# thiery-lab/manifold-mcmc-for-diffusions

Hardware: AMD Instinct MI355X
Metric: constrained-leapfrog steps/sec (all chains), FHN noisy-obs 400 sub-steps (higher is better)
Workload: dtype f64; 1 GPU; FHN noisy-obs, T=100 obs, S=400 steps/obs, R=5 obs/subseq, sigma_y=0.1, 256 chains per GPU (BASELINE.json configs[1]), Newton solver, standard splitting; chains_per_gpu=256, global_chains=256, dim_q=80106, traj_len=16, stepping=chmc_leapfrog_steps per trajectory (batched steps), chain_steps_nominal=152320, parallelism=chains x1 (no data-path collective, 1 gather), ranks_joined=1, collective_world_size=1, collective_route=torch.distributed gather, overlap_halves=-1

## Files before the change

### manifold_mcmc_for_diffusions_amd/context.py

```python
import ctypes as C
import numpy as np
from . import _lib
from ._lib import ChmcConfig, as_c, ptr, iptr, check

MODEL_IDS = {"fhn": 0, "sir": 1, "fhn_nb": 2}
STATUS_NAMES = {0: "ok", 1: "not_converged", 2: "diverged", 3: "non_reversible", -1: "inactive"}


class ChmcContext:
    def __init__(self, model, obs_interval, num_steps_per_obs, num_obs_per_subseq, y_seq, sigma=None,
                 use_gaussian_splitting=False, num_chains=1, device=0):
        L = _lib.lib()
        self.L = L
        y = as_c(np.asarray(y_seq).reshape(-1))
        self._y = y
        cfg = ChmcConfig(
            model=MODEL_IDS[model] if isinstance(model, str) else int(model), num_obs=len(y),
            num_steps_per_obs=int(num_steps_per_obs),
            num_obs_per_subseq=0 if num_obs_per_subseq is None else int(num_obs_per_subseq),
            noisy=2 if isinstance(sigma, str) else int(sigma is not None),
            use_gaussian_splitting=int(bool(use_gaussian_splitting)),
            num_chains=int(num_chains), device=int(device), obs_interval=float(obs_interval),
            sigma=0.0 if sigma is None or isinstance(sigma, str) else float(sigma), y_seq=ptr(y))
        h = C.c_void_p()
# ... 197 lines not shown
        check(self.L.chmc_jacob_constr_blocks(self.h, ptr(du), ptr(dv)), "chmc_jacob_constr_blocks")
        return du, dv

    def chol_gram_blocks(self):
        cC = np.empty((self.B, self.U, self.U))
        cD = np.empty((self.B, self.num_blocks, self.RM, self.RM))
        check(self.L.chmc_chol_gram_blocks(self.h, ptr(cC), ptr(cD)), "chmc_chol_gram_blocks")
        return cC, cD

    def log_det_sqrt_gram(self):
        out = np.empty(self.B)
        check(self.L.chmc_log_det_sqrt_gram(self.h, ptr(out)), "chmc_log_det_sqrt_gram")
        return out

    def grad_log_det_sqrt_gram(self):
        g = np.empty((self.B, self.Q))
        check(self.L.chmc_grad_log_det_sqrt_gram(self.h, ptr(g)), "chmc_grad_log_det_sqrt_gram")
        return g

    def lmult_by_jacob_constr(self, vct):
        vct = self._bq(vct, "vct")
        out = np.empty((self.B, self.dim_c))
        check(self.L.chmc_lmult_by_jacob_constr(self.h, ptr(vct), ptr(out)), "chmc_lmult_by_jacob_constr")
        return out

    def _bc(self, a, name):
        a = as_c(a)
        if a.shape != (self.B, self.dim_c):
            raise ValueError(f"{name} must have shape ({self.B}, {self.dim_c}), got {a.shape}")
        return a

    def rmult_by_jacob_constr(self, lam):
        lam = self._bc(lam, "vct")
        out = np.empty((self.B, self.Q))
        check(self.L.chmc_rmult_by_jacob_constr(self.h, ptr(lam), ptr(out)), "chmc_rmult_by_jacob_constr")
        return out

    def lmult_by_inv_gram(self, vct):
        vct = self._bc(vct, "vct")
        out = np.empty((self.B, self.dim_c))
        check(self.L.chmc_lmult_by_inv_gram(self.h, ptr(vct), ptr(out)), "chmc_lmult_by_inv_gram")
        return out

    def normal_space_component(self, vct):
        vct = self._bq(vct, "vct")
        out = np.empty((self.B, self.Q))
        check(self.L.chmc_normal_space_component(self.h, ptr(vct), ptr(out)), "chmc_normal_space_component")
        return out

    def project_onto_cotangent_space(self):
        check(self.L.chmc_project_onto_cotangent_space(self.h), "chmc_project_onto_cotangent_space")

    def hamiltonian(self):
        h = np.empty((self.B, 3))
        check(self.L.chmc_hamiltonian(self.h, ptr(h)), "chmc_hamiltonian")
        return h

    def neg_log_dens_and_grad(self, q, use_gaussian_splitting=False, want_grad=True):
        QH = self.U + self.NV
        q = as_c(q)
        if q.shape != (self.B, QH):
            raise ValueError(f"q must have shape ({self.B}, {QH}), got {q.shape}")
        val = np.empty(self.B)
        g = np.empty((self.B, QH)) if want_grad else None
        check(self.L.chmc_neg_log_dens_and_grad(self.h, ptr(q), int(bool(use_gaussian_splitting)), ptr(val), ptr(g)),
              "chmc_neg_log_dens_and_grad")
        return val, g

    def neg_log_dens_and_grad_device(self, q_dev_ptr, grad_dev_ptr=None, use_gaussian_splitting=False):
        val = np.empty(self.B)
        check(self.L.chmc_neg_log_dens_and_grad_device(self.h, C.c_void_p(q_dev_ptr), int(bool(use_gaussian_splitting)),
                                                       ptr(val), C.c_void_p(grad_dev_ptr or 0)),
              "chmc_neg_log_dens_and_grad_device")
        return val

    def adam_objective_device(self, u_v_dev_ptr, grad_dev_ptr):
        out = np.empty((self.B, 3))
        check(self.L.chmc_adam_objective_device(self.h, C.c_void_p(u_v_dev_ptr), C.c_void_p(grad_dev_ptr), ptr(out)),
              "chmc_adam_objective_device")
        return out

    def adam_update_device(self, u_v_dev_ptr, m_dev_ptr, v_dev_ptr, grad_dev_ptr, coef, b1=0.9, b2=0.999, eps=1e-8):
        coef = as_c(np.asarray(coef, dtype=np.float64).reshape(self.B, 2))
        check(self.L.chmc_adam_update_device(self.h, C.c_void_p(u_v_dev_ptr), C.c_void_p(m_dev_ptr), C.c_void_p(v_dev_ptr),
                                             C.c_void_p(grad_dev_ptr), ptr(coef), float(b1), float(b2), float(eps)),
              "chmc_adam_update_device")

    def project(self, q, dt, newton=True, constraint_tol=1e-9, position_tol=1e-8, divergence_tol=1e10, max_iters=50):
        q = self._bq(q, "q")
        dt = as_c(np.broadcast_to(np.asarray(dt, dtype=np.float64), (self.B,)))
        q_out, mu = np.empty((self.B, self.Q)), np.empty((self.B, self.Q))
        iters, status = np.zeros(self.B, dtype=np.int32), np.zeros(self.B, dtype=np.int32)
        ndq, err = np.empty(self.B), np.empty(self.B)
        check(self.L.chmc_project(self.h, int(newton), ptr(q), ptr(dt), constraint_tol, position_tol, divergence_tol,
                                  int(max_iters), ptr(q_out), ptr(mu), iptr(iters), ptr(ndq), ptr(err), iptr(status)),
              "chmc_project")
        return dict(q=q_out, mu=mu, iters=iters, norm_dq=ndq, err=err, status=status)

    def leapfrog_step(self, dt, active=None, n_inner_step=1, newton=True, constraint_tol=1e-9, position_tol=1e-8,
                      divergence_tol=1e10, max_iters=50, reverse_check_tol=2e-8):
        dt = as_c(np.broadcast_to(np.asarray(dt, dtype=np.float64), (self.B,)))
        act = None if active is None else np.ascontiguousarray(active, dtype=np.int32)
        status = np.zeros(self.B, dtype=np.int32)
        itf, itb = np.zeros(self.B, dtype=np.int32), np.zeros(self.B, dtype=np.int32)
        rev = np.zeros(self.B)
        check(self.L.chmc_leapfrog_step(self.h, ptr(dt), iptr(act), int(n_inner_step), int(newton), constraint_tol,
                                        position_tol, divergence_tol, int(max_iters), reverse_check_tol, iptr(status),
                                        iptr(itf), iptr(itb), ptr(rev)), "chmc_leapfrog_step")
        return dict(status=status, iters_fwd=itf, iters_bwd=itb, rev_err=rev)

    def leapfrog_steps(self, dt, n_steps, active=None, n_inner_step=1, newton=True, constraint_tol=1e-9, position_tol=1e-8,
                       divergence_tol=1e10, max_iters=50, reverse_check_tol=2e-8):
        dt = as_c(np.broadcast_to(np.asarray(dt, dtype=np.float64), (self.B,)))
        act = None if active is None else np.ascontiguousarray(active, dtype=np.int32)
        per_chain = None if np.isscalar(n_steps) else np.ascontiguousarray(np.broadcast_to(n_steps, (self.B,)), dtype=np.int32)
        n_all = int(n_steps) if per_chain is None else 0
        ndone, status = np.zeros(self.B, dtype=np.int32), np.zeros(self.B, dtype=np.int32)
        itf, itb = np.zeros(self.B, dtype=np.int32), np.zeros(self.B, dtype=np.int32)
        rev = np.zeros(self.B)
        check(self.L.chmc_leapfrog_steps(self.h, ptr(dt), iptr(act), iptr(per_chain), n_all, int(n_inner_step), int(newton),
                                         constraint_tol, position_tol, divergence_tol, int(max_iters), reverse_check_tol,
                                         iptr(ndone), iptr(status), iptr(itf), iptr(itb), ptr(rev)), "chmc_leapfrog_steps")
        return dict(n_done=ndone, status=status, iters_fwd=itf, iters_bwd=itb, rev_err=rev)

    def comm_init(self, id128, rank, world):
        buf = (C.c_char * 128).from_buffer_copy(bytes(id128))
        check(self.L.chmc_comm_init(self.h, buf, int(rank), int(world)), "chmc_comm_init")
        self.comm_world = int(world)

    @staticmethod
    def comm_unique_id():
        buf = (C.c_char * 128)()
        check(_lib.lib().chmc_comm_unique_id(buf), "chmc_comm_unique_id")
        return bytes(buf)

    def gather_samples_device(self, local_dev_ptr, count, gathered_dev_ptr):
        check(self.L.chmc_gather_samples(self.h, C.c_void_p(local_dev_ptr), int(count), C.c_void_p(gathered_dev_ptr)),
              "chmc_gather_samples")

    def comm_info(self):
        wd, rk = C.c_int(0), C.c_int(0)
        check(self.L.chmc_comm_info(self.h, C.byref(wd), C.byref(rk)), "chmc_comm_info")
        return wd.value, rk.value

    def comm_destroy(self):
        check(self.L.chmc_comm_destroy(self.h), "chmc_comm_destroy")

    def diagnostics(self):
        out = (C.c_longlong * 80)()
        check(self.L.chmc_get_diagnostics(self.h, out), "chmc_get_diagnostics")
        v = np.array(out[:], dtype=np.int64)
        return dict(par_scan=v[:64], gram_mfma_launches=int(v[64]), gram_valu_launches=int(v[65]),
                    retract_kernel_launches=int(v[66]), traj_kernel_launches=int(v[67]),
                    newton_fsm_launches=int(v[68]), newton_factor8_launches=int(v[69]), extra=v[68:80])

    def counters(self):
        out = (C.c_longlong * 8)()
        check(self.L.chmc_get_counters(self.h, out), "chmc_get_counters")
        keys = ("constr", "jacob_constr_blocks", "lu_jacob_product_blocks", "chol_gram_blocks",
                "grad_log_det_sqrt_gram", "leapfrog_step", "projection_iterations", "_")
        return dict(zip(keys, (int(v) for v in out)))
```

### manifold_mcmc_for_diffusions_amd/csrc/chmc_api.inc

```
#include <string>
#include <algorithm>
#include <vector>
#include <cstring>
#include <cstdio>
#include <cstdlib>
#include <cmath>
#include <thread>
#include <type_traits>
#include "../../include/chmc.h"
#include "chmc_plan.h"
#include "chmc_layout.h"

using namespace chmc;

static thread_local std::string g_err;
static int fail(const std::string& m) {
  g_err = m;
  return -1;
}
#include CHMC_BACKEND_HEADER

struct chmc_ctx : ChainView {
  std::thread::id owner = std::this_thread::get_id();
  chmc_config cfg;
  int model, RMt, part, num_partition, npart_sum;
  int K[2], C[2];
  std::vector<BlockDesc> hblk[2];
  BlockDesc* d_blk[2];
  int* d_obs2blk[2];
  int* d_order[2];
  double *d_y, *d_ham;
  unsigned long long* d_out = nullptr;
  BlockDesc* d_blk_full = nullptr;
  int* d_order_ident = nullptr;
  bool mom_tangent = false;
  bool snap_tangent = false;
  bool have_state = false;
  double* d_m0 = nullptr;
  double *d_tree_part = nullptr, *d_tree_out = nullptr;
  int* d_tree_mask = nullptr;
  TreeState tree{};
  bool have_tree = false;
  bool rows_fresh = false;
  std::vector<unsigned char> h_out;
  std::vector<void*> allocs;
  long long counters[8];
  PlanInput plan_in{};
  KernelPlan plan{};
  long long diag[16] = {0};
  int round = 0;
  int halves = 1;
  int hB[2] = {0, 0}, hc0[2] = {0, 0};
  int* d_order_half[2][2] = {{nullptr, nullptr}, {nullptr, nullptr}};
  void* comm = nullptr;
  int comm_rank = 0, comm_world = 1;
  int last_n_inner = 1;
  int proj_rounds[2] = {0, 0}, proj_stable[2] = {0, 0};
  int num_cus = 256;
  std::vector<double> last_dt;
  std::vector<int> last_active;
  bool last_active_null = true;
};

template <class T_>
static T_* alloc(chmc_ctx* c, size_t n) {
  T_* p = (T_*)dev_alloc(n * sizeof(T_));
  c->allocs.push_back(p);
  return p;
}
static void alloc_chain_arrays(chmc_ctx* c) {
  const size_t B = c->sy.B;
  for_each_chain_array(*c, c->plan, c->npart_sum, [&](auto*& p, size_t per_chain, int kind, size_t slack) {
    using T_ = std::remove_reference_t<decltype(*p)>;
    p = nullptr;
    if (kind & (kLazy | kAbsent)) return;
    p = alloc<T_>(c, B * per_chain + slack);
    if (kind & kZeroed) dev_zero(p, sizeof(T_) * (B * per_chain + slack));
  });
}
template <class T_>
static void ensure_array(chmc_ctx* c, T_*& want) {
  if (want) return;
  const size_t B = c->sy.B;
  for_each_chain_array(*c, c->plan, c->npart_sum, [&](auto*& p, size_t per_chain, int, size_t slack) {
    if ((void*)&p == (void*)&want) want = alloc<T_>(c, B * per_chain + slack);
  });
}

static int* upload_work_order(chmc_ctx* c, const std::vector<BlockDesc>& blk, int chains, int slack) {
  const int K = (int)blk.size();
  std::vector<int> order((size_t)chains * K);
  for (size_t i = 0; i < order.size(); ++i) order[i] = (int)i;
  std::stable_sort(order.begin(), order.end(), [&](int a, int b) { return blk[a % K].nsteps > blk[b % K].nsteps; });
  int* d = alloc<int>(c, order.size() + slack);
  if (!order.empty()) h2d(d, order.data(), sizeof(int) * order.size());
  return d;
}

static void build_partition(chmc_ctx* c, int p, int init) {
  const chmc_config& g = c->cfg;
  const int T = g.num_obs, R = g.num_obs_per_subseq, S = g.num_steps_per_obs;
  const int X = c->sy.X, V = c->sy.V, V0 = c->sy.V0;
  std::vector<int> sizes;
  if (R <= 0 || R >= T) {
    sizes.push_back(T);
  } else {
    int num_full = (T - init) / R, num_rem = (T - init) % R;
    int num_middle = num_rem == 0 ? num_full - 1 : num_full;
    int final_ = num_rem == 0 ? R : num_rem;
    sizes.push_back(init);
    for (int i = 0; i < num_middle; ++i) sizes.push_back(R);
    sizes.push_back(final_);
  }
  int obs = 0, row = 0;
  for (size_t b = 0; b < sizes.size(); ++b) {
    BlockDesc B;
    memset(&B, 0, sizeof(B));
    B.obs0 = obs, B.nobs = sizes[b], B.first = b == 0, B.last = b + 1 == sizes.size();
    B.ny = (B.last || g.noisy) ? B.nobs : B.nobs - 1;
    B.nrows = B.ny + (B.last ? 0 : X);
    B.row0 = row;
    B.step0 = obs * S, B.nsteps = B.nobs * S;
    B.col0 = B.first ? 0 : V0 + B.step0 * V;
    B.ncols = B.nsteps * V + (B.first ? V0 : 0);
    row += B.nrows, obs += B.nobs;
    c->hblk[p].push_back(B);
  }
  c->K[p] = (int)sizes.size();
  c->C[p] = row;
}

using ViewSave = ChainView;
static ViewSave save_view(const chmc_ctx* c) { return *c; }
static void restore_view(chmc_ctx* c, const ViewSave& f) { static_cast<ChainView&>(*c) = f; }
static void set_half(chmc_ctx* c, const ViewSave& f, int h) {
  const size_t c0 = (size_t)c->hc0[h];
  ChainView& v = *c;
  v = f;
  for_each_chain_array(v, c->plan, c->npart_sum, [&](auto*& p, size_t per_chain, int, size_t) {
    if (p) p += c0 * per_chain;
  });
  alias_step_outputs(v, c->d_out, f.sy.B, c0);
  v.sy.B = c->hB[h];
  v.sy.xobs = v.d_xobs;
  v.sy.order = c->d_order_half[c->part][h];
  v.w.n_active = f.w.n_active + 4 * (1 + h);
  use_stream(h);
}

static void select_partition(chmc_ctx* c, int p) {
  c->part = p;
  c->sy.K = c->K[p];
  c->sy.C = c->C[p];
  c->sy.blk = c->d_blk[p];
  c->sy.obs2blk = c->d_obs2blk[p];
  c->sy.order = c->d_order[p];
}

#define CHMC_DISPATCH(ctx, ...)                   \
  do {                                            \
    if ((ctx)->sy.varsig) {  \
      if ((ctx)->model == CHMC_MODEL_FHN) {       \
        using M = FhnVsModel;                     \
        constexpr int RM = 8;                     \
        __VA_ARGS__                               \
      } else if ((ctx)->RMt == 8) {               \
        using M = SirVsModel;                     \
        constexpr int RM = 8;                     \
        __VA_ARGS__                               \
      } else {                                    \
        using M = SirVsModel;                     \
        constexpr int RM = 16;                    \
        __VA_ARGS__                               \
      }                                           \
    } else if ((ctx)->model == CHMC_MODEL_FHN) {  \
      using M = FhnModel;                         \
      if ((ctx)->RMt == 7) {                      \
        constexpr int RM = 7;                     \
        __VA_ARGS__                               \
      } else if ((ctx)->RMt == 6) {               \
        constexpr int RM = 6;                     \
        __VA_ARGS__                               \
      } else {                                    \
        constexpr int RM = 8;                     \
        __VA_ARGS__                               \
      }                                           \
    } else if ((ctx)->model == CHMC_MODEL_FHN_NOTEBOOK) { \
      using M = FhnNbModel;                       \
      if ((ctx)->RMt == 6) {                      \
        constexpr int RM = 6;                     \
        __VA_ARGS__                               \
      } else {                                    \
        constexpr int RM = 8;                     \
        __VA_ARGS__                               \
      }                                           \
    } else if ((ctx)->RMt == 8) {                 \
      using M = SirModel;                         \
      constexpr int RM = 8;                       \
      __VA_ARGS__                                 \
    } else {                                      \
      using M = SirModel;                         \
      constexpr int RM = 16;                      \
      __VA_ARGS__                                 \
    }                                             \
  } while (0)

static const PartitionPlan& part_plan(const chmc_ctx* c) { return c->plan.part[c->part]; }
static void refresh_plan(chmc_ctx* c) {
  c->plan_in.call = read_switches();
  c->plan = make_plan(c->plan_in);
}
#ifdef CHMC_WAVE_KERNELS
#define CHMC_SOLVE_CHAIN(T1, T2, T3, T4, ...)                                                   \
  do {                                                                                          \
    if (sy.K <= 64)                                                                             \
      launch_wave(k_solve_chain_wave<T1, T2, T3, T4>, (long)sy.B, 5, __VA_ARGS__);              \
    else                                                                                        \
      launch(KSolveChain<T1, T2, T3, T4>{__VA_ARGS__}, sy.B, 5);                                \
  } while (0)
#else
#define CHMC_SOLVE_CHAIN(T1, T2, T3, T4, ...) launch(KSolveChain<T1, T2, T3, T4>{__VA_ARGS__}, sy.B, 5)
#endif

#ifdef CHMC_WAVE_KERNELS
#define CHMC_FWD_PAR(W_, N_, ...)                                                        \
  do {                                                                                   \
    if ((W_) == 8)                                                                       \
      launch_blocks(k_fwd_par<M, RM, 8>, N_, 512, 7, __VA_ARGS__);                       \
    else if ((W_) == 4)                                                                  \
      launch_blocks(k_fwd_par<M, RM, 4>, N_, 256, 7, __VA_ARGS__);                       \
    else if ((W_) == 2)                                                                  \
      launch_blocks(k_fwd_par<M, RM, 2>, N_, 128, 7, __VA_ARGS__);                       \
    else                                                                                 \
      launch_blocks(k_fwd_par<M, RM, 1>, N_, 64, 7, __VA_ARGS__);                        \
  } while (0)
#define CHMC_FWD(WHICH_, QSEL_, USENW_, STORE_, GSEL_)                                                           \
  do {                                                                                                           \
    stagger_wait();                   \
    const FwdScan fwd_ = (GSEL_) != 0 ? c->plan.fwd : c->plan.fwd_cold;                                          \
    if (fwd_ == FwdPar) {                                                                                        \
       \
                                                             \
      CHMC_FWD_PAR(c->plan.fwd_waves, (long)sy.B * sy.K, sy, c->sl, c->w, WHICH_, QSEL_, USENW_,                 \
                   (STORE_) ? (STORE_) : 2, GSEL_, c->round);                                                    \
    } else if (fwd_ == FwdWave) {                                                                                \
      if (STORE_)                                                                                                \
        launch_blocks(k_fwd_scan<M, RM, true>, ((long)sy.B * sy.K + 63) / 64, 64 * (1 + CHMC_SCAN_HELPERS), 7, sy, c->sl, c->w, WHICH_,   \
                      QSEL_, USENW_, STORE_);                                                                    \
      else                                                                                                       \
        launch_blocks(k_fwd_scan<M, RM, false>, ((long)sy.B * sy.K + 63) / 64, 64, 7, sy, c->sl, c->w, WHICH_,   \
                      QSEL_, USENW_, STORE_);                                                                    \
    } else {                                                                                                     \
      launch(KFwd<M, RM>{sy, c->sl, c->w, WHICH_, QSEL_, USENW_, STORE_}, (long)sy.B * sy.K, 7);                 \
    }                                                                                                            \
    stagger_record();                                                                                            \
  } while (0)
#else
#define CHMC_FWD(WHICH_, QSEL_, USENW_, STORE_, GSEL_) \
  launch(KFwd<M, RM>{sy, c->sl, c->w, WHICH_, QSEL_, USENW_, STORE_}, (long)sy.B * sy.K, 7)
#endif

#define CHMC_UPDATE_PB(TGT_, WHICH_, QSEL_, PSEL_)                                                                \
  do {                                                                                                           \
    launch(KMuF<RM, M::X, TGT_>{sy, c->sl, c->w, WHICH_}, (long)sy.B * sy.K * sy.NOBS * M::X, 5);                 \
    launch_colmax(KUpdatePB<RM, M::X, M::V, TGT_, 1>{sy, c->sl, c->w, WHICH_, QSEL_, PSEL_},                      \
                  sy.T * sy.S + sy.V0 + (sy.noisy ? sy.T : 0), sy.B, 4);                                         \
  } while (0)

#define CHMC_UPDATE(TGT_, ...)                                                                         \
  do {                                                                                                 \
    if (sy.Q % 2 == 0 && sy.NV % 2 == 0 && sy.U % 2 == 0 && sy.V0 % 2 == 0 && sy.V % 2 == 0 &&         \
        sy.NCOL % 2 == 0)                                                                              \
      launch_colmax(KUpdate<RM, TGT_, 2>{__VA_ARGS__}, sy.NCOL / 2, sy.B, 4);                          \
    else                                                                                               \
      launch_colmax(KUpdate<RM, TGT_, 1>{__VA_ARGS__}, sy.NCOL, sy.B, 4);                              \
  } while (0)

extern "C" const char* chmc_last_error(void) { return g_err.c_str(); }
extern "C" const char* chmc_backend(void) { return CHMC_BACKEND_NAME; }

extern "C" int chmc_create(const chmc_config* cfg, chmc_ctx** out) {
  if (!cfg || !out) return fail("chmc_create: null argument");
  if (cfg->model != CHMC_MODEL_FHN && cfg->model != CHMC_MODEL_SIR && cfg->model != CHMC_MODEL_FHN_NOTEBOOK)
    return fail("chmc_create: unknown model id");
  if (cfg->num_obs < 1 || cfg->num_steps_per_obs < 1 || cfg->num_chains < 1) return fail("chmc_create: bad sizes");
  if (!cfg->y_seq) return fail("chmc_create: y_seq is null");
  if (cfg->noisy == 1 && !(cfg->sigma > 0.0)) return fail("chmc_create: noisy observations need sigma > 0");
  if (cfg->noisy < 0 || cfg->noisy > 2) return fail("chmc_create: noisy must be 0 (noiseless), 1 (fixed sigma) or 2 (sigma = generate_sigma(u))");
  if (cfg->noisy == 2 && cfg->model == CHMC_MODEL_FHN_NOTEBOOK)
    return fail("chmc_create: the notebook model has no generate_sigma (noiseless observations)");
  if (cfg->num_obs_per_subseq == 1 && cfg->num_obs > 1)
    return fail("chmc_create: num_obs_per_subseq must be at least 2 (or <= 0 / >= num_obs for a single sub-sequence)");
  if (dev_init(cfg->device)) return fail(std::string("chmc_create: ") + g_err);
  chmc_ctx* c = new chmc_ctx();
  c->num_cus = dev_num_cus();
  c->cfg = *cfg;
  c->cfg.y_seq = nullptr;
  c->model = cfg->model;
  memset(c->counters, 0, sizeof(c->counters));
  Sys& sy = c->sy;
  memset(&sy, 0, sizeof(sy));
  const bool fhn = cfg->model == CHMC_MODEL_FHN || cfg->model == CHMC_MODEL_FHN_NOTEBOOK;
  sy.X = fhn ? FhnModel::X : SirModel::X, sy.V = fhn ? FhnModel::V : SirModel::V;
  sy.Z = fhn ? FhnModel::Z : SirModel::Z, sy.V0 = fhn ? FhnModel::V0 : SirModel::V0;
  sy.varsig = cfg->noisy == 2;
  sy.U = sy.Z + sy.varsig;
  sy.B = cfg->num_chains, sy.T = cfg->num_obs, sy.S = cfg->num_steps_per_obs;
  sy.noisy = cfg->noisy != 0, sy.gaussian = cfg->use_gaussian_splitting != 0;
  sy.dl = cfg->obs_interval / cfg->num_steps_per_obs;
  sy.sigma = cfg->noisy == 1 ? cfg->sigma : 0.0;
  sy.NV = sy.V0 + sy.T * sy.S * sy.V;
  sy.NCOL = sy.NV + (sy.noisy ? sy.T : 0);
  sy.Q = sy.U + sy.NCOL;
  const int R = cfg->num_obs_per_subseq;
  if (R <= 0 || R >= sy.T) {
    c->num_partition = 1;
    build_partition(c, 0, sy.T);
  } else {
    c->num_partition = 2;
    build_partition(c, 0, R);
    build_partition(c, 1, R / 2);
  }
  int rmax = 0, kmax = 0, nobsmax = 1;
  for (int p = 0; p < c->num_partition; ++p) {
    for (auto& b : c->hblk[p]) {
      rmax = b.nrows > rmax ? b.nrows : rmax;
      nobsmax = b.nobs > nobsmax ? b.nobs : nobsmax;
    }
    kmax = c->K[p] > kmax ? c->K[p] : kmax;
  }
  sy.NOBS = nobsmax;
  if (rmax > 16 || (fhn && rmax > 8)) {
    delete c;
    return fail("chmc_create: blocks with more than 8 (FHN) / 16 (SIR) constraint rows are not supported");
  }
  c->RMt = rmax <= 8 ? 8 : 16;
  if (fhn && !sy.varsig && (rmax == 6 || (rmax == 7 && cfg->model == CHMC_MODEL_FHN))) c->RMt = rmax;
  sy.RM = c->RMt, sy.Kmax = kmax, sy.TRJ = (sy.T * sy.S + CHMC_TPAD * kmax) * sy.X;
  const size_t B = sy.B;
  c->hB[0] = sy.B / 2, c->hB[1] = sy.B - sy.B / 2, c->hc0[0] = 0, c->hc0[1] = sy.B / 2;
  for (int p = 0; p < c->num_partition; ++p) {
    c->d_blk[p] = alloc<BlockDesc>(c, c->K[p]);
    h2d(c->d_blk[p], c->hblk[p].data(), sizeof(BlockDesc) * c->K[p]);
    std::vector<int> o2b(sy.T);
    for (int b = 0; b < c->K[p]; ++b)
      for (int t = 0; t < c->hblk[p][b].nobs; ++t) o2b[c->hblk[p][b].obs0 + t] = b;
    c->d_obs2blk[p] = alloc<int>(c, sy.T);
    h2d(c->d_obs2blk[p], o2b.data(), sizeof(int) * sy.T);
    c->d_order[p] = upload_work_order(c, c->hblk[p], sy.B, 0);
    for (int h = 0; h < 2; ++h) c->d_order_half[p][h] = upload_work_order(c, c->hblk[p], c->hB[h], 1);
  }
  {
    PlanInput& in = c->plan_in;
    in.rmt = c->RMt, in.num_partition = c->num_partition, in.K[0] = c->K[0], in.K[1] = c->K[c->num_partition - 1];
    in.longest = 0;
    for (int p = 0; p < c->num_partition; ++p)
      for (auto& bl : c->hblk[p]) in.longest = bl.nsteps > in.longest ? bl.nsteps : in.longest;
    in.chain_steps = sy.T * sy.S, in.s_tiles8 = sy.S % 8 == 0;
    in.V = sy.V, in.even_dims = !((sy.Q | sy.U | sy.V0 | sy.NV) & 1), in.gaussian = sy.gaussian;
#ifdef CHMC_WAVE_KERNELS
    in.wave_kernels = true;
#endif
    in.sw = in.call = read_switches();
    c->plan = make_plan(in);
  }
  {
    c->halves = (c->plan_in.sw.halves == 2 && sy.B >= 2) ? 2 : 1;
    if (kmax == 1 && (c->plan.par_scan || c->RMt > 8)) c->halves = 1;
  }
  c->d_y = alloc<double>(c, sy.T);
  h2d(c->d_y, cfg->y_seq, sizeof(double) * sy.T);
  c->npart_sum = rowsum_groups(sy.Q);
  alloc_chain_arrays(c);
  sy.y = c->d_y, sy.xobs = c->d_xobs;
  c->d_out = alloc<unsigned long long>(c, step_outputs_words(B));
  alias_step_outputs(*c, c->d_out, B, 0);
  Work& w = c->w;
  w.n_active = alloc<int>(c, 12);
  {
    double* z = alloc<double>(c, 256);
    dev_zero(z, sizeof(double) * 256);
    w.zeros = z;
  }
  w.nfallback = alloc<int>(c, 128);
  dev_zero(w.nfallback, sizeof(int) * 128);
  c->d_ham = alloc<double>(c, B * 4);
  select_partition(c, 0);
  if (dev_sync()) {
    std::string e = g_err;
    chmc_destroy(c);
    return fail("chmc_create: " + e);
  }
  *out = c;
  return 0;
}

extern "C" int chmc_comm_destroy(chmc_ctx* ctx);
extern "C" void chmc_destroy(chmc_ctx* c) {
  if (!c) return;
  if (c->comm) chmc_comm_destroy(c);
  for (void* p : c->allocs) dev_free(p);
  delete c;
}

extern "C" int chmc_get_dims(const chmc_ctx* c, int* d) {
  if (!c || !d) return fail("chmc_get_dims: null argument");
  const Sys& s = c->sy;
  int v[16] = {s.B, s.Q, s.NV, s.U, s.X, s.T, s.S, c->num_partition, s.RM, s.Kmax,
               c->C[0], c->num_partition > 1 ? c->C[1] : 0, c->K[0], c->num_partition > 1 ? c->K[1] : 0, s.V, s.V0};
  memcpy(d, v, sizeof(v));
  return 0;
}
extern "C" int chmc_get_blocks(const chmc_ctx* c, int p, int* out) {
  if (!c || !out || p < 0 || p >= c->num_partition) return fail("chmc_get_blocks: bad argument");
  memcpy(out, c->hblk[p].data(), sizeof(BlockDesc) * c->K[p]);
  return 0;
}
extern "C" int chmc_get_counters(const chmc_ctx* c, long long* out8) {
  if (!c || !out8) return fail("chmc_get_counters: null argument");
  memcpy(out8, c->counters, sizeof(c->counters));
  return 0;
}

static void begin_all(chmc_ctx* c, const double* d_dt, const int* d_active, double dt_scale = 1.0) {
  launch(KBegin{c->w, d_active, d_dt, dt_scale}, c->sy.B);
}

static void ensure_rows(chmc_ctx* c) {
#ifdef CHMC_WAVE_KERNELS
  if (!part_plan(c).rebuild_rows || c->rows_fresh) return;
  const Sys& sy = c->sy;
  CHMC_DISPATCH(c, {
    launch(KRowsFromPB<RM, M::X, M::V>{sy, c->sl}, (long)sy.B * sy.T * sy.S, 2);
  });
  c->rows_fresh = true;
#else
  (void)c;
#endif
}
static void state_eval_core(chmc_ctx* c, int which, bool with_grad = true, int traj_guess = 0) {
  const Sys& sy = c->sy;
  const PartitionPlan& pp = part_plan(c);
  (void)pp;
  c->rows_fresh = false;
  CHMC_DISPATCH(c, {
#ifdef CHMC_WAVE_KERNELS
    CHMC_FWD(which, 0, 0, 1, traj_guess);
    const long nbk = (long)sy.B * sy.K;
    if constexpr (RM > 8) {
      switch (pp.state) {
        case StateIvlComb:
          launch_blocks(k_newton_ivl<M, true>, nbk * sy.NOBS, 64, 2, sy, c->sl, c->w, which, 0);
          launch_blocks(k_newton_comb<M, RM, true>, nbk, 64, 2, sy, c->sl, c->w, which, 0);
          break;
        case StateIvlCombWg:
          launch_blocks(k_newton_ivl<M, true>, nbk * sy.NOBS, 64, 2, sy, c->sl, c->w, which, 0);
          launch_blocks(k_newton_comb_wg<M, RM, CHMC_RETRACT_WAVES, true>, (long)sy.B, 64 * CHMC_RETRACT_WAVES, 2, sy, c->sl,
                        c->w, which, 0);
          break;
        case StateLdsrowsGramMfma:
          launch_blocks(k_rev_wave_ldsrows<M, RM, 0>, nbk, 64, 2, sy, c->sl, c->w, which, 0);
          launch_blocks(k_gram_rows_mfma<RM>, nbk, 64, 2, sy, c->sl, c->w, which, 0, 0), c->diag[0]++;
          break;
        default:
          launch_blocks(k_rev_wave_ldsrows<M, RM, 0>, nbk, 64, 2, sy, c->sl, c->w, which, 0);
          launch_wave(k_gram_rows<RM, 4>, nbk * (RM / 4), 2, sy, c->sl, c->w, which, 0, 0), c->diag[1]++;
      }
    } else {
      switch (pp.state) {
        case StateLean:
          launch_blocks(k_newton_lean<M, RM, true, true>, nbk, 64, 2, sy, c->sl, c->w, which, 0);
          break;
        case StateRevStoreGramMfma:
          launch_wave(k_rev_wave<M, RM, 0, false>, nbk, 2, sy, c->sl, c->w, which, 0);
          launch_blocks(k_gram_rows_mfma<RM>, nbk, 64, 2, sy, c->sl, c->w, which, 0, 0), c->diag[0]++;
          break;
        default:
          launch_wave(k_rev_wave<M, RM, 0>, nbk, 2, sy, c->sl, c->w, which, 0);
      }
    }
    if (pp.state != StateIvlCombWg)
      launch(KStateFactor<M, RM>{sy, c->sl, c->w, which}, nbk, 9);
#else
    launch(KStateBlk<M, RM>{sy, c->sl, c->w, which}, (long)sy.B * sy.K, 2);
#endif
    launch(KStateChain<M>{sy, c->sl, c->w, which}, sy.B);
    if (!with_grad) break;
#ifdef CHMC_WAVE_KERNELS
    if constexpr (RM > 8)
      launch_blocks(k_gld_prep_wave<M, RM>, ((long)sy.B * sy.K + 3) / 4, 64, 9, sy, c->sl, c->w, which);
    else
      launch(KGldPrep<M, RM>{sy, c->sl, c->w, which}, (long)sy.B * sy.K, 9);
    switch (pp.gld) {
      case GldQxLean:
        if constexpr (RM <= 8) {
          launch_wave(k_gld_fwd_qx<M, RM>, nbk, 3, sy, c->sl, c->w, which);
          launch_blocks(k_gld_bwd_lean<M, RM>, nbk, 64, 3, sy, c->sl, c->w, which);
        }
        break;
      case GldIvl:
        if constexpr (RM > 8) {
          const long niv = nbk * sy.NOBS;
          launch_wave(k_gld_ivl_prologue<M, RM>, nbk, 3, sy, c->sl, c->w, which);
          launch_wave(k_gld_fwd_ivl<M, RM>, niv, 3, sy, c->sl, c->w, which);
          launch_wave(k_gld_bwd_ivl<M, RM, 0>, niv, 3, sy, c->sl, c->w, which);
          launch_wave(k_gld_bwd_ivl<M, RM, 1>, niv, 3, sy, c->sl, c->w, which);
          launch_blocks(k_gld_ivl_finish<M, RM>, (nbk + 63) / 64, 64, 3, sy, c->sl, c->w, which);
        }
        break;
      case GldCompactFwdStored:
        if constexpr (RM > 8) {
          launch_wave(k_gld_fwd_wave<M, RM, true, false>, nbk, 3, sy, c->sl, c->w, which);
          launch_wave(k_gld_bwd_wave_ldsrows<M, RM>, nbk, 3, sy, c->sl, c->w, which);
        }
        break;
      case GldStored:
        launch_wave(k_gld_fwd_wave<M, RM>, nbk, 3, sy, c->sl, c->w, which);
        if constexpr (RM > 8) {
          launch_wave(k_gld_bwd_wave_ldsrows<M, RM>, nbk, 3, sy, c->sl, c->w, which);
        } else {
          launch_wave(k_gld_bwd_wave<M, RM>, nbk, 3, sy, c->sl, c->w, which);
        }
        break;
    }
#else
    launch(KGldBlk<M, RM>{sy, c->sl, c->w, which}, (long)sy.B * sy.K, 3);
#endif
    launch(KGldChain<M>{sy, c->sl, c->w, which}, sy.B);
  });
  c->counters[0]++, c->counters[1]++, c->counters[3]++, c->counters[4] += with_grad ? 1 : 0;
}

static void project_momentum(chmc_ctx* c, int which, int vsel, int psel);
static void state_eval(chmc_ctx* c, int which) {
  const Sys& sy = c->sy;
  state_eval_core(c, which);
  launch(KInitPg{sy, c->sl, c->w, which}, (long)sy.B * sy.Q, 8);
  project_momentum(c, which, 4, 3);
}
static void project_momentum_and_kick_direction(chmc_ctx* c, int which, bool init_pg, bool fix_in_jw = false,
                                                bool flow_rev = false) {
  const Sys& sy = c->sy;
  if (init_pg) launch(KInitPg{sy, c->sl, c->w, which}, (long)sy.B * sy.Q, 8);
#ifdef CHMC_WAVE_KERNELS
  CHMC_DISPATCH(c, {
    const bool compact = c->plan.rows == RowsCompact;
    switch (part_plan(c).jp) {
      case JpPbWg:
        if constexpr (RM > 8)
          launch_blocks(k_jw_pb_wg<RM, M::X, M::V, CHMC_RETRACT_WAVES>, (long)sy.B, 64 * CHMC_RETRACT_WAVES, 6, sy, c->sl, c->w,
                        which);
        break;
      case JpPb:
        if constexpr (RM <= 8 && M::V == 2) {
          if (fix_in_jw) {
            launch_wave(k_jw_pb<RM, M::X, M::V, true, true>, (long)sy.B * sy.K, 6, sy, c->sl, c->w, which, 256);
            break;
          }
        }
        launch_wave(k_jw_pb<RM, M::X, M::V, true>, (long)sy.B * sy.K, 6, sy, c->sl, c->w, which, 256);
        break;
      case JpWave:
        launch_wave(k_jw_wave<RM, true>, (long)sy.B * sy.K, 6, sy, c->sl, c->w, which, 256);
        break;
    }
    Work w1 = c->w, w2 = c->w;
    w1.lampad = c->w.lampad2;
    w2.cpad = c->w.cpad2;
    launch(KSymBlk<M, RM>{sy, c->sl, w1, which, 0}, (long)sy.B * sy.K, 9);
    CHMC_SOLVE_CHAIN(M, RM, 1, 1, sy, c->sl, w1, which, 0, 0);
    launch(KSymBlk<M, RM>{sy, c->sl, w2, which, 0}, (long)sy.B * sy.K, 9);
    CHMC_SOLVE_CHAIN(M, RM, 1, 1, sy, c->sl, w2, which, 0, 3);
    if (compact && flow_rev) {
      launch(KMuF<RM, M::X, 3>{sy, c->sl, c->w, which}, (long)sy.B * sy.K * sy.NOBS * M::X, 5);
      launch_colmax(KUpdatePB<RM, M::X, M::V, 3, 1>{sy, c->sl, c->w, which, 0, 0, 1},
                    sy.T * sy.S + sy.V0 + (sy.noisy ? sy.T : 0), sy.B, 4);
    } else if (compact) {
      CHMC_UPDATE_PB(3, which, 0, 0);
    } else {
      CHMC_UPDATE(3, sy, c->sl, c->w, which, 0, 0);
    }
  });
#else
  (void)fix_in_jw, (void)flow_rev;
  project_momentum(c, which, 0, 0);
  project_momentum(c, which, 4, 3);
#endif
}

static void project_momentum(chmc_ctx* c, int which, int vsel, int psel) {
  const Sys& sy = c->sy;
  CHMC_DISPATCH(c, {
    const bool compact = c->plan.rows == RowsCompact;
#ifdef CHMC_WAVE_KERNELS
    if (compact)
      launch_wave(k_jw_pb<RM, M::X, M::V>, (long)sy.B * sy.K, 6, sy, c->sl, c->w, which, vsel | 256);
    else
      launch_wave(k_jw_wave<RM>, (long)sy.B * sy.K, 6, sy, c->sl, c->w, which, vsel | 256);
#else
    launch(KJw<RM>{sy, c->sl, c->w, which, vsel | 256}, (long)sy.B * sy.K * RM, 6);
#endif
    launch(KSymBlk<M, RM>{sy, c->sl, c->w, which, 0}, (long)sy.B * sy.K, 9);
    CHMC_SOLVE_CHAIN(M, RM, 1, 1, sy, c->sl, c->w, which, 0, psel);
    if (compact) {
      CHMC_UPDATE_PB(1, which, 0, psel);
    } else {
      CHMC_UPDATE(1, sy, c->sl, c->w, which, 0, psel);
    }
  });
}

static void iteration_scan(chmc_ctx* c, int newton, int prev, int qsel, int fwd_guess, int use_nw) {
  const Sys& sy = c->sy;
  CHMC_DISPATCH(c, {
    if (newton) {
#ifdef CHMC_WAVE_KERNELS
      CHMC_FWD(prev ^ 1, qsel, use_nw, 2, fwd_guess);
#else
      (void)fwd_guess, (void)use_nw;
#endif
    } else {
      CHMC_FWD(prev ^ 1, qsel, use_nw, 0, fwd_guess);
    }
  });
}
static void iteration_after_scan(chmc_ctx* c, int newton, int prev, int qsel) {
  const Sys& sy = c->sy;
  const NewtonSweep sweep = part_plan(c).newton;
  const bool solved = newton && (sweep == NewtonIvlFsm || sweep == Newton16IvlCombFactor || sweep == Newton16IvlCombWg);
  CHMC_DISPATCH(c, {
    if (newton) {
#ifdef CHMC_WAVE_KERNELS
      const long nbk = (long)sy.B * sy.K;
      if constexpr (RM > 8) {
        switch (sweep) {
          case Newton16IvlCombWg:
            launch_blocks(k_newton_ivl<M>, nbk * sy.NOBS, 64, 1, sy, c->sl, c->w, prev, qsel);
            launch_blocks(k_newton_comb_wg<M, RM, CHMC_RETRACT_WAVES, false>, (long)sy.B, 64 * CHMC_RETRACT_WAVES, 1, sy,
                          c->sl, c->w, prev, qsel);
            break;
          case Newton16IvlCombFactor:
            launch_blocks(k_newton_ivl<M>, nbk * sy.NOBS, 64, 1, sy, c->sl, c->w, prev, qsel);
            launch_blocks(k_newton_comb<M, RM, false, true>, nbk, 64, 1, sy, c->sl, c->w, prev, qsel);
            break;
          case Newton16IvlComb:
            launch_blocks(k_newton_ivl<M>, nbk * sy.NOBS, 64, 1, sy, c->sl, c->w, prev, qsel);
            launch_blocks(k_newton_comb<M, RM>, nbk, 64, 1, sy, c->sl, c->w, prev, qsel);
            break;
          case Newton16LdsrowsGramMfma:
            launch_blocks(k_rev_wave_ldsrows<M, RM, 1>, nbk, 64, 1, sy, c->sl, c->w, prev, qsel);
            launch_blocks(k_gram_rows_mfma<RM>, nbk, 64, 1, sy, c->sl, c->w, prev, 1, qsel), c->diag[0]++;
            break;
          default:
            launch_blocks(k_rev_wave_ldsrows<M, RM, 1>, nbk, 64, 1, sy, c->sl, c->w, prev, qsel);
            launch_wave(k_gram_rows<RM, 4>, nbk * (RM / 4), 1, sy, c->sl, c->w, prev, 1, qsel), c->diag[1]++;
        }
        if (!solved) launch_blocks(k_newton_factor_wave<M, RM>, (nbk + 3) / 4, 64, 9, sy, c->sl, c->w, prev, qsel);
      } else {
        switch (sweep) {
          case NewtonIvlFsm:
          case NewtonIvlComb:
            launch_blocks(k_newton_ivl<M>, nbk * sy.NOBS, 64, 1, sy, c->sl, c->w, prev, qsel);
            launch_blocks(k_newton_comb<M, RM>, nbk, 64, 1, sy, c->sl, c->w, prev, qsel);
            break;
          case NewtonRevStoreGramMfma:
            launch_wave(k_rev_wave<M, RM, 1, false>, nbk, 1, sy, c->sl, c->w, prev, qsel);
            launch_blocks(k_gram_rows_mfma<RM>, nbk, 64, 1, sy, c->sl, c->w, prev, 1, qsel), c->diag[0]++;
            break;
          default:
            launch_wave(k_rev_wave<M, RM, 1>, nbk, 1, sy, c->sl, c->w, prev, qsel);
        }
        if (solved)
          launch_blocks(k_newton_fsm_wave<M, RM>, (long)sy.B, 64, 5, sy, c->sl, c->w, prev, qsel), c->diag[4]++;
        else
          launch(KNewtonFactor<M, RM>{sy, c->sl, c->w, prev}, nbk, 9), c->diag[5]++;
      }
#else
      launch(KNewtonBlk<M, RM>{sy, c->sl, c->w, prev, qsel}, (long)sy.B * sy.K, 1);
#endif
      if (!solved) CHMC_SOLVE_CHAIN(M, RM, 0, 0, sy, c->sl, c->w, prev, qsel, 0);
    } else {
      launch(KSymBlk<M, RM>{sy, c->sl, c->w, prev, 1}, (long)sy.B * sy.K, 9);
      CHMC_SOLVE_CHAIN(M, RM, 1, 0, sy, c->sl, c->w, prev, qsel, 0);
    }
#ifdef CHMC_WAVE_KERNELS
    if (c->plan.rows == RowsCompact) {
      if (!solved) launch(KMuF<RM, M::X, 0>{sy, c->sl, c->w, prev}, (long)sy.B * sy.K * sy.NOBS * M::X, 5);
      launch_colmax(KUpdatePB<RM, M::X, M::V, 0, 1>{sy, c->sl, c->w, prev, qsel, 0},
                    sy.T * sy.S + sy.V0 + (sy.noisy ? sy.T : 0), sy.B, 4);
    } else
#endif
    CHMC_UPDATE(0, sy, c->sl, c->w, prev, qsel, 0);
  });
}

static int retract_waves(const chmc_ctx* c, int newton, const void* views) {
  return chain_kernel_waves(c->plan, part_plan(c).retract_chain, c->sy.B, c->num_cus, newton != 0, views != nullptr);
}
static int traj_waves(const chmc_ctx* c, int n_inner, int newton) {
  const bool eligible = part_plan(c).traj_chain && n_inner == 1 && c->mom_tangent && c->halves == 1;
  return chain_kernel_waves(c->plan, eligible, c->sy.B, c->num_cus, newton != 0, false);
}
static int run_projection(chmc_ctx* c, int newton, int prev, int qsel, double ctol, double ptol, double dtol,
                          int max_iters, const ViewSave* views = nullptr, int count_dir = -1) {
  const Sys& sy = c->sy;
#ifdef CHMC_WAVE_KERNELS
  if (const int waves = retract_waves(c, newton, views)) {
    int* iters_dst = count_dir < 0 ? nullptr : (count_dir ? c->d_itb : c->d_itf);
    CHMC_DISPATCH(c, {
      if constexpr (RM == 16) {
        if (waves == 4)
          launch_blocks(k_retract_chain<M, RM, 4>, (long)sy.B, 256, 1, sy, c->sl, c->w, prev, qsel, ctol, ptol, dtol, max_iters,
                        iters_dst);
        else
          launch_blocks(k_retract_chain<M, RM, CHMC_RETRACT_WAVES>, (long)sy.B, 64 * CHMC_RETRACT_WAVES, 1, sy, c->sl, c->w, prev,
                        qsel, ctol, ptol, dtol, max_iters, iters_dst);
      }
    });
    c->counters[6]++;
    c->diag[2]++;
    return 0;
  }
#endif
  const int nh = views ? 2 : 1;
  auto enter = [&](int h) {
    if (views) set_half(c, *views, h);
  };
  for (int h = 0; h < nh; ++h) {
    enter(h);
    if (sy.B > 0) launch(KNewtonBegin{c->w}, sy.B);
  }
  int fwd_guess = 2;
#ifdef CHMC_WAVE_KERNELS
  const bool carry = c->plan.par_scan && sy.K == 1;
#else
  const bool carry = false;
#endif
  const int max_rounds = carry ? 12 * (max_iters + 1) : max_iters;
  auto iteration = [&](int poll_slot) {
    iteration_scan(c, newton, prev, qsel, fwd_guess, 1);
    iteration_after_scan(c, newton, prev, qsel);
    const KCheck chk{c->w, ctol, ptol, dtol, max_iters, sy.B, count_dir < 0 ? nullptr : (count_dir ? c->d_itb : c->d_itf),
                     c->round & 3};
    if (poll_slot >= 0) launch_publish(chk, sy.B, c->w.n_active + (c->round & 3), poll_slot);
    else launch(chk, sy.B);
  };
  bool done[2] = {false, nh == 1};
  for (int h = 0; h < nh; ++h) {
    enter(h);
    if (sy.B <= 0) done[h] = true;
  }
  int& expect = c->proj_rounds[prev & 1];
  int& stable = c->proj_stable[prev & 1];
  const bool predict = !views && stable >= 3 && expect >= 2;
  int rounds_done = 0;
  for (int it = 0; it < max_rounds && !(done[0] && done[1]); ++it) {
    if (predict && it >= expect && poll_end((it - 1) & 1) == 0) {
      done[0] = true;
      break;
    }
    for (int h = 0; h < nh; ++h) {
      if (done[h]) continue;
      enter(h);
      fwd_guess = it == 0 ? 2 : 1;
      c->round = it;
      iteration(it >= 1 ? 2 * h + (it & 1) : -1);
    }
    c->counters[6]++;
    if (it == 0) continue;
    bool all_empty = true;
    for (int h = 0; h < nh; ++h) {
      if (done[h]) continue;
      if (it >= 2 && poll_end(2 * h + ((it - 1) & 1)) == 0) {
        done[h] = true;
        continue;
      }
      all_empty = false;
      if (it + 1 >= max_rounds) poll_end(2 * h + (it & 1));
    }
    if (all_empty) c->counters[6]--;
    else rounds_done = it + 1;
  }
  if (!views) {
    if (predict && done[0] && rounds_done < expect) rounds_done = expect;
    stable = rounds_done == expect ? stable + 1 : 0;
    expect = rounds_done;
  }
  for (int h = 0; h < nh; ++h) {
    enter(h);
    if (sy.B > 0) launch(KNewtonEnd{c->w, count_dir < 0 ? nullptr : (count_dir ? c->d_itb : c->d_itf)}, sy.B);
  }
  c->round = 0;
  return 0;
}

static int check_ctx(const chmc_ctx* c, const char* fn) {
  if (!c) return fail(std::string(fn) + ": null context");
  if (c->owner != std::this_thread::get_id())
    return fail(std::string(fn) + ": a context must be driven by the host thread that created it");
  return 0;
}
#define CHMC_ENTER(fn)                 \
  if (check_ctx(ctx, fn)) return -1;   \
  refresh_plan(ctx);                   \
  use_stream(-1);                      \
  if (dev_set(ctx->cfg.device)) return fail(std::string(fn) + ": " + g_err);
#define CHMC_LEAVE(fn)                                                 \
  if (dev_sync()) return fail(std::string(fn) + ": " + g_err);        \
  return 0;

extern "C" int chmc_get_diagnostics(chmc_ctx* ctx, long long* out80) {
  CHMC_ENTER("chmc_get_diagnostics")
  if (!out80) return fail("chmc_get_diagnostics: null output");
  int ps[80];
  d2h(ps, ctx->w.nfallback, sizeof(ps));
  for (int i = 0; i < 64; ++i) out80[i] = ps[i];
  for (int i = 0; i < 16; ++i) out80[64 + i] = ctx->diag[i];
#ifdef CHMC_RETRACT_PROF
  for (int i = 4; i < 16; ++i) out80[64 + i] = ps[64 + i - 4];
#endif
  CHMC_LEAVE("chmc_get_diagnostics")
}

extern "C" int chmc_set_state(chmc_ctx* ctx, const double* q, const double* p, const double* x_obs, int partition) {
  CHMC_ENTER("chmc_set_state")
  if (!q || !x_obs) return fail("chmc_set_state: q and x_obs_seq are required");
  if (partition < 0 || partition >= ctx->num_partition) return fail("chmc_set_state: partition out of range");
  const Sys& sy = ctx->sy;
  const size_t n = sizeof(double) * (size_t)sy.B * sy.Q;
  dev_zero(ctx->sl.cur, sizeof(int) * sy.B);
  h2d(ctx->sl.q[0], q, n);
  if (p) h2d(ctx->sl.p[0], p, n);
  else dev_zero(ctx->sl.p[0], n);
  h2d(ctx->d_xobs, x_obs, sizeof(double) * (size_t)sy.B * sy.T * sy.X);
  select_partition(ctx, partition);
  begin_all(ctx, nullptr, nullptr);
  state_eval(ctx, 0);
  ctx->have_state = true;
  ctx->mom_tangent = p == nullptr;
  CHMC_LEAVE("chmc_set_state")
}

extern "C" int chmc_init_linear_interpolation(chmc_ctx* ctx, const double* u, const double* v_0,
                                              const double* x_obs_seq_init, int partition) {
  CHMC_ENTER("chmc_init_linear_interpolation")
  if (!u || !v_0 || !x_obs_seq_init) return fail("chmc_init_linear_interpolation: u, v_0 and x_obs_seq_init are required");
  if (partition < 0 || partition >= ctx->num_partition)
    return fail("chmc_init_linear_interpolation: partition out of range");
  const Sys& sy = ctx->sy;
  double* d_u = ctx->w.pb;
  double* d_v0 = ctx->w.pb + (size_t)sy.B * sy.U;
  h2d(d_u, u, sizeof(double) * (size_t)sy.B * sy.U);
  h2d(d_v0, v_0, sizeof(double) * (size_t)sy.B * sy.V0);
  h2d(ctx->d_xobs, x_obs_seq_init, sizeof(double) * (size_t)sy.B * sy.T * sy.X);
  dev_zero(ctx->sl.cur, sizeof(int) * sy.B);
  dev_zero(ctx->sl.p[0], sizeof(double) * (size_t)sy.B * sy.Q);
  if (ctx->model == CHMC_MODEL_FHN)
    launch(KInitInterp<FhnModel>{sy, ctx->sl.q[0], d_u, d_v0, ctx->d_xobs}, (long)sy.B * sy.T * sy.S);
  else if (ctx->model == CHMC_MODEL_FHN_NOTEBOOK)
    launch(KInitInterp<FhnNbModel>{sy, ctx->sl.q[0], d_u, d_v0, ctx->d_xobs}, (long)sy.B * sy.T * sy.S);
  else
    launch(KInitInterp<SirModel>{sy, ctx->sl.q[0], d_u, d_v0, ctx->d_xobs}, (long)sy.B * sy.T * sy.S);
  select_partition(ctx, partition);
  begin_all(ctx, nullptr, nullptr);
  state_eval(ctx, 0);
  ctx->have_state = true;
  ctx->mom_tangent = true;
  CHMC_LEAVE("chmc_init_linear_interpolation")
}

struct KGatherState {
  Sys sy;
  Slots sl;
  double *qo, *po;
  CHMC_HD void operator()(int tid) const {
    const int c = tid / sy.Q;
    const int s = sl.cur[c];
    if (qo) qo[tid] = pick(sl.q, s)[tid];
    if (po) po[tid] = pick(sl.p, s)[tid];
  }
};
struct KScatterMom {
  Sys sy;
  Slots sl;
  const double* pi;
  CHMC_HD void operator()(int tid) const {
    const int c = tid / sy.Q;
    sl.p[sl.cur[c]][tid] = pi[tid];
  }
};
struct KGatherSlotVec {
  Slots sl;
  const double* a0;
  const double* a1;
  double* out;
  long stride;
  CHMC_HD void operator()(int tid) const {
    const int c = (int)(tid / stride);
    out[tid] = (sl.cur[c] ? a1 : a0)[tid];
  }
};

extern "C" int chmc_get_state(chmc_ctx* ctx, double* q, double* p, double* x_obs, int* partition) {
  CHMC_ENTER("chmc_get_state")
  const Sys& sy = ctx->sy;
  const size_t n = sizeof(double) * (size_t)sy.B * sy.Q;
  launch(KGatherState{sy, ctx->sl, q ? ctx->w.qb : nullptr, p ? ctx->w.pb : nullptr}, (long)sy.B * sy.Q);
  if (q) d2h(q, ctx->w.qb, n);
  if (p) d2h(p, ctx->w.pb, n);
  if (x_obs) d2h(x_obs, ctx->d_xobs, sizeof(double) * (size_t)sy.B * sy.T * sy.X);
  if (partition) *partition = ctx->part;
  CHMC_LEAVE("chmc_get_state")
}
extern "C" int chmc_get_state_device(chmc_ctx* ctx, void* q_dev, void* p_dev) {
  CHMC_ENTER("chmc_get_state_device")
  const Sys& sy = ctx->sy;
  launch(KGatherState{sy, ctx->sl, (double*)q_dev, (double*)p_dev}, (long)sy.B * sy.Q);
  CHMC_LEAVE("chmc_get_state_device")
}
extern "C" int chmc_set_momentum(chmc_ctx* ctx, const double* p) {
  CHMC_ENTER("chmc_set_momentum")
  if (!p) return fail("chmc_set_momentum: null momentum");
  const Sys& sy = ctx->sy;
  h2d(ctx->w.pb, p, sizeof(double) * (size_t)sy.B * sy.Q);
  launch(KScatterMom{sy, ctx->sl, ctx->w.pb}, (long)sy.B * sy.Q);
  ctx->mom_tangent = false;
  CHMC_LEAVE("chmc_set_momentum")
}
extern "C" int chmc_set_momentum_device(chmc_ctx* ctx, const void* p_dev) {
  CHMC_ENTER("chmc_set_momentum_device")
  if (!p_dev) return fail("chmc_set_momentum_device: null momentum");
  const Sys& sy = ctx->sy;
  launch(KScatterMom{sy, ctx->sl, (const double*)p_dev}, (long)sy.B * sy.Q);
  ctx->mom_tangent = false;
  CHMC_LEAVE("chmc_set_momentum_device")
}

extern "C" int chmc_set_metric(chmc_ctx* ctx, const double* M0) {
  CHMC_ENTER("chmc_set_metric")
  Sys& sy = ctx->sy;
  const int U = sy.U;
  if (!M0) {
    sy.m0 = nullptr, sy.hld_m0 = 0.0;
  } else {
// ... 233 lines not shown
    unpad_rows(ctx, pad, dc_du, sy.U);
  }
  if (dc_dv) {
    ensure_rows(ctx);
    std::vector<int> cur(sy.B);
    d2h(cur.data(), ctx->sl.cur, sizeof(int) * sy.B);
    const size_t st = (size_t)sy.RM * sy.NV;
    for (int ch = 0; ch < sy.B; ++ch) d2h(dc_dv + ch * st, ctx->sl.Jv[cur[ch]] + ch * st, sizeof(double) * st);
  }
  CHMC_LEAVE("chmc_jacob_constr_blocks")
}
extern "C" int chmc_chol_gram_blocks(chmc_ctx* ctx, double* chol_C, double* chol_D) {
  CHMC_ENTER("chmc_chol_gram_blocks")
  const Sys& sy = ctx->sy;
  std::vector<int> cur(sy.B);
  d2h(cur.data(), ctx->sl.cur, sizeof(int) * sy.B);
  for (int ch = 0; ch < sy.B; ++ch) {
    if (chol_C)
      d2h(chol_C + (size_t)ch * sy.U * sy.U, ctx->sl.facC[cur[ch]] + (size_t)ch * sy.U * sy.U, sizeof(double) * sy.U * sy.U);
    if (chol_D)
      for (int b = 0; b < sy.K; ++b)
        d2h(chol_D + ((size_t)ch * sy.K + b) * sy.RM * sy.RM,
            ctx->sl.facD[cur[ch]] + ((size_t)ch * sy.Kmax + b) * sy.RM * sy.RM, sizeof(double) * sy.RM * sy.RM);
  }
  CHMC_LEAVE("chmc_chol_gram_blocks")
}
extern "C" int chmc_log_det_sqrt_gram(chmc_ctx* ctx, double* out) {
  CHMC_ENTER("chmc_log_det_sqrt_gram")
  if (!out) return fail("chmc_log_det_sqrt_gram: null output");
  fetch_slot(ctx, ctx->sl.logdet, out, 1, ctx->w.err);
  CHMC_LEAVE("chmc_log_det_sqrt_gram")
}
extern "C" int chmc_grad_log_det_sqrt_gram(chmc_ctx* ctx, double* grad) {
  CHMC_ENTER("chmc_grad_log_det_sqrt_gram")
  if (!grad) return fail("chmc_grad_log_det_sqrt_gram: null output");
  fetch_slot(ctx, ctx->sl.grad, grad, ctx->sy.Q, ctx->w.qb);
  CHMC_LEAVE("chmc_grad_log_det_sqrt_gram")
}
extern "C" int chmc_lmult_by_jacob_constr(chmc_ctx* ctx, const double* vct, double* out) {
  CHMC_ENTER("chmc_lmult_by_jacob_constr")
  if (!vct || !out) return fail("chmc_lmult_by_jacob_constr: null argument");
  const Sys& sy = ctx->sy;
  ensure_rows(ctx);
  h2d(ctx->w.vin, vct, sizeof(double) * (size_t)sy.B * sy.Q);
  begin_all(ctx, nullptr, nullptr);
#ifdef CHMC_WAVE_KERNELS
  CHMC_DISPATCH(ctx, { launch_wave(k_jw_wave<RM>, (long)sy.B * sy.K, 6, sy, ctx->sl, ctx->w, 0, 2); });
#else
  CHMC_DISPATCH(ctx, { launch(KJw<RM>{sy, ctx->sl, ctx->w, 0, 2}, (long)sy.B * sy.K * RM, 6); });
#endif
  fetch_padded(ctx, ctx->w.cpad, out, 1);
  CHMC_LEAVE("chmc_lmult_by_jacob_constr")
}
struct KJtLamU {
  Sys sy;
  Slots sl;
  Work w;
  CHMC_HD void operator()(int c) const {
    const int s = sl.cur[c];
    for (int a = 0; a < sy.U; ++a) {
      double t = 0.0;
      for (int b = 0; b < sy.K; ++b)
        for (int i = 0; i < sy.RM; ++i)
          t += pick(sl.JuP, s)[(((size_t)c * sy.Kmax + b) * sy.RM + i) * sy.U + a] * w.lampad[((size_t)c * sy.Kmax + b) * sy.RM + i];
      w.pb[(size_t)c * sy.Q + a] = t;
    }
  }
};
extern "C" int chmc_rmult_by_jacob_constr(chmc_ctx* ctx, const double* vct, double* out) {
  CHMC_ENTER("chmc_rmult_by_jacob_constr")
  if (!vct || !out) return fail("chmc_rmult_by_jacob_constr: null argument");
  const Sys& sy = ctx->sy;
  ensure_rows(ctx);
  std::vector<double> pad;
  pad_rows(ctx, vct, pad);
  h2d(ctx->w.lampad, pad.data(), sizeof(double) * pad.size());
  begin_all(ctx, nullptr, nullptr);
  CHMC_DISPATCH(ctx, { CHMC_UPDATE(2, sy, ctx->sl, ctx->w, 0, 0, 0); });
  launch(KJtLamU{sy, ctx->sl, ctx->w}, sy.B);
  d2h(out, ctx->w.pb, sizeof(double) * (size_t)sy.B * sy.Q);
  CHMC_LEAVE("chmc_rmult_by_jacob_constr")
}
extern "C" int chmc_lmult_by_inv_gram(chmc_ctx* ctx, const double* vct, double* out) {
  CHMC_ENTER("chmc_lmult_by_inv_gram")
  if (!vct || !out) return fail("chmc_lmult_by_inv_gram: null argument");
  const Sys& sy = ctx->sy;
  std::vector<double> pad;
  pad_rows(ctx, vct, pad);
  h2d(ctx->w.cpad, pad.data(), sizeof(double) * pad.size());
  begin_all(ctx, nullptr, nullptr);
  CHMC_DISPATCH(ctx, {
    launch(KSymBlk<M, RM>{sy, ctx->sl, ctx->w, 0, 0}, (long)sy.B * sy.K, 9);
    CHMC_SOLVE_CHAIN(M, RM, 1, 2, sy, ctx->sl, ctx->w, 0, 0, 0);
  });
  fetch_padded(ctx, ctx->w.lampad, out, 1);
  CHMC_LEAVE("chmc_lmult_by_inv_gram")
}
extern "C" int chmc_normal_space_component(chmc_ctx* ctx, const double* vct, double* out) {
  CHMC_ENTER("chmc_normal_space_component")
  if (!vct || !out) return fail("chmc_normal_space_component: null argument");
  const Sys& sy = ctx->sy;
  ensure_rows(ctx);
  h2d(ctx->w.vin, vct, sizeof(double) * (size_t)sy.B * sy.Q);
  begin_all(ctx, nullptr, nullptr);
  CHMC_DISPATCH(ctx, {
#ifdef CHMC_WAVE_KERNELS
    launch_wave(k_jw_wave<RM>, (long)sy.B * sy.K, 6, sy, ctx->sl, ctx->w, 0, 2 | 256);
#else
    launch(KJw<RM>{sy, ctx->sl, ctx->w, 0, 2 | 256}, (long)sy.B * sy.K * RM, 6);
#endif
    launch(KSymBlk<M, RM>{sy, ctx->sl, ctx->w, 0, 0}, (long)sy.B * sy.K, 9);
    CHMC_SOLVE_CHAIN(M, RM, 1, 2, sy, ctx->sl, ctx->w, 0, 0, 0);
    CHMC_UPDATE(2, sy, ctx->sl, ctx->w, 0, 0, 0);
  });
  launch(KJtLamU{sy, ctx->sl, ctx->w}, sy.B);
  d2h(out, ctx->w.pb, sizeof(double) * (size_t)sy.B * sy.Q);
  CHMC_LEAVE("chmc_normal_space_component")
}
extern "C" int chmc_project_onto_cotangent_space(chmc_ctx* ctx) {
  CHMC_ENTER("chmc_project_onto_cotangent_space")
  begin_all(ctx, nullptr, nullptr);
  project_momentum(ctx, 0, 0, 0);
  ctx->mom_tangent = true;
  CHMC_LEAVE("chmc_project_onto_cotangent_space")
}
static int nld_core(chmc_ctx* ctx, int use_gaussian_splitting, double* grad_dev) {
#ifdef CHMC_WAVE_KERNELS
  const Sys& sy = ctx->sy;
  const int QH = sy.U + sy.NV;
  Sys sf = sy;
  if (!ctx->d_blk_full) {
    BlockDesc bf{};
    bf.obs0 = 0, bf.nobs = sy.T, bf.first = 1, bf.last = 1, bf.row0 = 0, bf.nrows = 0, bf.ny = 0;
    bf.col0 = 0, bf.ncols = sy.NV, bf.step0 = 0, bf.nsteps = sy.T * sy.S;
    ctx->d_blk_full = alloc<BlockDesc>(ctx, 1);
    h2d(ctx->d_blk_full, &bf, sizeof(BlockDesc));
  }
  sf.K = 1, sf.Kmax = 1, sf.Q = QH, sf.blk = ctx->d_blk_full;
  const bool par = ctx->plan.nld == FwdPar;
  if (par && !ctx->d_order_ident) {
    std::vector<int> id(sy.B);
    for (int i = 0; i < sy.B; ++i) id[i] = i;
    ctx->d_order_ident = alloc<int>(ctx, sy.B);
    h2d(ctx->d_order_ident, id.data(), sizeof(int) * sy.B);
  }
  begin_all(ctx, nullptr, nullptr);
  CHMC_DISPATCH(ctx, {
    (void)RM;
    if (par) {
      Sys sp = sf;
      sp.order = ctx->d_order_ident;
      CHMC_FWD_PAR(ctx->plan.nld_waves, (long)sy.B, sp, ctx->sl, ctx->w, 0, 1, 0, 2, 1, 0);
    } else if (ctx->plan.nld == FwdWave)
      launch_blocks(k_fwd_scan<M, RM, true>, ((long)sy.B + 63) / 64, 64 * (1 + CHMC_SCAN_HELPERS), 7, sf, ctx->sl, ctx->w, 0, 1, 0, 2);
    else
      launch(KFullScan<M>{sy, ctx->w.qb, ctx->w.trajw, QH}, sy.B, 7);
    launch_wave(k_nld_grad_wave<M>, (long)sy.B, 0, sy, ctx->w.qb, ctx->w.trajw, QH, use_gaussian_splitting, ctx->d_ham,
                grad_dev);
  });
  return 0;
#else
  (void)ctx, (void)use_gaussian_splitting, (void)grad_dev;
  return fail("chmc_neg_log_dens_and_grad: not available in the host emulation build");
#endif
}
extern "C" int chmc_neg_log_dens_and_grad(chmc_ctx* ctx, const double* q, int use_gaussian_splitting, double* value,
                                          double* grad) {
  CHMC_ENTER("chmc_neg_log_dens_and_grad")
  const Sys& sy = ctx->sy;
  if (!q || !value) return fail("chmc_neg_log_dens_and_grad: q and value are required");
  if (!sy.noisy) return fail("chmc_neg_log_dens_and_grad: needs observation noise (the density is degenerate without)");
  const size_t n = sizeof(double) * (size_t)sy.B * (sy.U + sy.NV);
  h2d(ctx->w.qb, q, n);
  if (nld_core(ctx, use_gaussian_splitting, grad ? ctx->w.pb : nullptr)) return -1;
  d2h(value, ctx->d_ham, sizeof(double) * sy.B);
  if (grad) d2h(grad, ctx->w.pb, n);
  CHMC_LEAVE("chmc_neg_log_dens_and_grad")
}
extern "C" int chmc_neg_log_dens_and_grad_device(chmc_ctx* ctx, const void* q_dev, int use_gaussian_splitting,
                                                 double* value, void* grad_dev) {
  CHMC_ENTER("chmc_neg_log_dens_and_grad_device")
  const Sys& sy = ctx->sy;
  if (!q_dev || !value) return fail("chmc_neg_log_dens_and_grad_device: q_dev and value are required");
  if (!sy.noisy) return fail("chmc_neg_log_dens_and_grad_device: needs observation noise (the density is degenerate without)");
  d2d(ctx->w.qb, q_dev, sizeof(double) * (size_t)sy.B * (sy.U + sy.NV));
  if (nld_core(ctx, use_gaussian_splitting, (double*)grad_dev)) return -1;
  d2h(value, ctx->d_ham, sizeof(double) * sy.B);
  CHMC_LEAVE("chmc_neg_log_dens_and_grad_device")
}
extern "C" int chmc_adam_objective_device(chmc_ctx* ctx, const void* u_v_dev, void* grad_dev, double* out3) {
  CHMC_ENTER("chmc_adam_objective_device")
  const Sys& sy = ctx->sy;
  if (!u_v_dev || !grad_dev || !out3) return fail("chmc_adam_objective_device: null argument");
  if (!sy.noisy) return fail("chmc_adam_objective_device: needs observation noise");
  const int n = sy.U + sy.NV;
  d2d(ctx->w.qb, u_v_dev, sizeof(double) * (size_t)sy.B * n);
  if (nld_core(ctx, 0, (double*)grad_dev)) return -1;
  launch_rowsum(KAdamRow{(const double*)u_v_dev, (const double*)grad_dev, n}, n, sy.B, 2, ctx->w.part, 8);
  launch(KAdamStats{ctx->w.part, ctx->d_ham, rowsum_groups(n), ctx->d_ham + sy.B}, sy.B);
  d2h(out3, ctx->d_ham + sy.B, sizeof(double) * (size_t)sy.B * 3);
  CHMC_LEAVE("chmc_adam_objective_device")
}
extern "C" int chmc_adam_update_device(chmc_ctx* ctx, void* u_v_dev, void* m_dev, void* v_dev, const void* grad_dev,
                                       const double* coef, double b1, double b2, double eps) {
  CHMC_ENTER("chmc_adam_update_device")
  const Sys& sy = ctx->sy;
  if (!u_v_dev || !m_dev || !v_dev || !grad_dev || !coef) return fail("chmc_adam_update_device: null argument");
  const int n = sy.U + sy.NV;
  h2d(ctx->d_ham, coef, sizeof(double) * (size_t)sy.B * 2);
  launch(KAdamUpdate{(double*)u_v_dev, (double*)m_dev, (double*)v_dev, (const double*)grad_dev, ctx->d_ham, n, b1, b2, eps},
         (long)sy.B * n, 8);
  CHMC_LEAVE("chmc_adam_update_device")
}
extern "C" int chmc_hamiltonian(chmc_ctx* ctx, double* h) {
  CHMC_ENTER("chmc_hamiltonian")
  if (!h) return fail("chmc_hamiltonian: null output");
  const Sys& sy = ctx->sy;
  launch_rowsum(KNormRow{sy, ctx->sl}, sy.Q, sy.B, 2, ctx->w.part, 8);
  launch(KHamiltonian{sy, ctx->sl, ctx->w, ctx->npart_sum, ctx->d_ham}, sy.B);
  d2h(h, ctx->d_ham, sizeof(double) * (size_t)sy.B * 3);
  CHMC_LEAVE("chmc_hamiltonian")
}

struct KMuFromMove {
  Sys sy;
  Slots sl;
  Work w;
  const double* q_in;
  CHMC_HD void operator()(int tid) const {
    const int c = tid / sy.Q;
    const double dt = w.dt[c];
    const int col = tid - c * sy.Q;
    double d = q_in[tid] - sl.q[sl.cur[c] ^ 1][tid];
    if (sy.m0 && col < sy.U) {
      d = 0.0;
      for (int b = 0; b < sy.U; ++b)
        d += sy.m0[col * sy.U + b] * (q_in[(size_t)c * sy.Q + b] - sl.q[sl.cur[c] ^ 1][(size_t)c * sy.Q + b]);
    }
    w.mu[tid] = d / (sy.gaussian ? sin(dt) : dt);
  }
};
struct KCopyToOther {
  Sys sy;
  Slots sl;
  const double* src;
  CHMC_HD void operator()(int tid) const {
    const int c = tid / sy.Q;
    sl.q[sl.cur[c] ^ 1][tid] = src[tid];
  }
};
struct KGatherOtherQ {
  Sys sy;
  Slots sl;
  double* out;
  CHMC_HD void operator()(int tid) const {
    const int c = tid / sy.Q;
    out[tid] = sl.q[sl.cur[c] ^ 1][tid];
  }
};

extern "C" int chmc_project(chmc_ctx* ctx, int newton, const double* q, const double* dt, double ctol, double ptol,
                            double dtol, int max_iters, double* q_out, double* mu_out, int* iters, double* norm_dq,
                            double* err, int* status) {
  CHMC_ENTER("chmc_project")
  if (!q || !dt) return fail("chmc_project: q and dt are required");
  if (max_iters < 0) return fail("chmc_project: max_iters < 0");
  const Sys& sy = ctx->sy;
  const size_t n = sizeof(double) * (size_t)sy.B * sy.Q;
  h2d(ctx->w.vin, q, n);
  h2d(ctx->w.err, dt, sizeof(double) * sy.B);
  ctx->last_dt.clear();
  begin_all(ctx, ctx->w.err, nullptr);
  launch(KCopyToOther{sy, ctx->sl, ctx->w.vin}, (long)sy.B * sy.Q);
  run_projection(ctx, newton, 0, 0, ctol, ptol, dtol, max_iters);
  if (mu_out) {
    launch(KMuFromMove{sy, ctx->sl, ctx->w, ctx->w.vin}, (long)sy.B * sy.Q);
    d2h(mu_out, ctx->w.mu, n);
  }
  if (q_out) {
    launch(KGatherOtherQ{sy, ctx->sl, ctx->w.vin}, (long)sy.B * sy.Q);
    d2h(q_out, ctx->w.vin, n);
  }
  if (iters) d2h(iters, ctx->w.iters, sizeof(int) * sy.B);
  if (err) d2h(err, ctx->w.err, sizeof(double) * sy.B);
  if (norm_dq) d2h(norm_dq, ctx->w.ndq, sizeof(double) * sy.B);
  if (status) d2h(status, ctx->w.nstat, sizeof(int) * sy.B);
  CHMC_LEAVE("chmc_project")
}

struct KInnerRestore {
  Sys sy;
  Slots sl;
  const double *q0, *p0;
  const int* mask;
  CHMC_HD void operator()(int tid) const {
    const int c = tid / sy.Q;
    if (!mask[c]) return;
    const int s = sl.cur[c];
    pick(sl.q, s)[tid] = q0[tid];
    pick(sl.p, s)[tid] = p0[tid];
  }
};

static int step_enqueue(chmc_ctx* ctx, const double* dt, const int* active, const int* active_dev, int n_inner, int newton,
                        double ctol, double ptol, double dtol, int max_iters, double rev_tol,
                        const int* n_steps_host = nullptr, int n_steps_all = 1, bool want_n_done = false,
                        bool skip_end_kick = false, bool pending_kick = false) {
  const Sys& sy = ctx->sy;
  const double* d_dt = nullptr;
  if (ctx->last_dt.size() != (size_t)sy.B || ctx->last_n_inner != n_inner ||
      memcmp(ctx->last_dt.data(), dt, sizeof(double) * sy.B) != 0) {
    h2d(ctx->w.err, dt, sizeof(double) * sy.B);
    ctx->last_dt.assign(dt, dt + sy.B);
    ctx->last_n_inner = n_inner;
    d_dt = ctx->w.err;
  }
  const int* d_active = nullptr;
  if (active_dev) {
    d2d(ctx->d_act, active_dev, sizeof(int) * sy.B);
    ctx->last_active_null = true;
    ctx->last_active.clear();
    d_active = ctx->d_act;
  } else if (active) {
    if (ctx->last_active_null || memcmp(ctx->last_active.data(), active, sizeof(int) * sy.B) != 0) {
      h2d(ctx->d_act, active, sizeof(int) * sy.B);
      ctx->last_active.assign(active, active + sy.B);
      ctx->last_active_null = false;
    }
    d_active = ctx->d_act;
  } else {
    ctx->last_active_null = true;
  }
  if (n_inner > 1) ensure_array(ctx, ctx->d_q0), ensure_array(ctx, ctx->d_p0), ensure_array(ctx, ctx->d_ncommit);
#ifdef CHMC_WAVE_KERNELS
  if (const int waves = traj_waves(ctx, n_inner, newton)) {
    ensure_array(ctx, ctx->d_nsteps), ensure_array(ctx, ctx->d_ndone);
    if (n_steps_host) h2d(ctx->d_nsteps, n_steps_host, sizeof(int) * sy.B);
    begin_all(ctx, d_dt ? ctx->w.err : nullptr, d_active ? ctx->d_act : nullptr, 1.0);
    dev_zero(ctx->d_itf, sizeof(int) * sy.B), dev_zero(ctx->d_itb, sizeof(int) * sy.B);
    CHMC_DISPATCH(ctx, {
      if constexpr (RM == 16) {
        if (waves == 4)
          launch_blocks(k_traj_chain<M, RM, 4>, (long)sy.B, 256, 1, sy, ctx->sl, ctx->w,
                        n_steps_host ? ctx->d_nsteps : nullptr, n_steps_all, ctol, ptol, dtol, max_iters, rev_tol, ctx->d_itf,
                        ctx->d_itb, want_n_done ? ctx->d_ndone : nullptr);
        else
          launch_blocks(k_traj_chain<M, RM, CHMC_RETRACT_WAVES>, (long)sy.B, 64 * CHMC_RETRACT_WAVES, 1, sy, ctx->sl, ctx->w,
                        n_steps_host ? ctx->d_nsteps : nullptr, n_steps_all, ctol, ptol, dtol, max_iters, rev_tol, ctx->d_itf,
                        ctx->d_itb, want_n_done ? ctx->d_ndone : nullptr);
      }
    });
    ctx->rows_fresh = false;
    ctx->diag[3]++;
    const int ns = n_steps_host ? 1 : n_steps_all;
    ctx->counters[0] += ns, ctx->counters[1] += ns, ctx->counters[3] += ns, ctx->counters[4] += ns, ctx->counters[6] += 2 * ns;
    return 0;
  }
#endif
  const bool two = ctx->halves == 2;
  const ViewSave full = save_view(ctx);
  const int nh = two ? 2 : 1;
  const double kick = 0.5 * n_inner;
  auto enter = [&](int h) {
    if (two) set_half(ctx, full, h);
  };
  if (two) streams_fork();
  for (int h = 0; h < nh; ++h) {
    enter(h);
    begin_all(ctx, d_dt ? ctx->w.err : nullptr, d_active ? ctx->d_act : nullptr, 1.0 / n_inner);
    dev_zero(ctx->d_itf, sizeof(int) * sy.B), dev_zero(ctx->d_itb, sizeof(int) * sy.B);
    if (n_inner > 1) {
      dev_zero(ctx->d_ncommit, sizeof(int) * sy.B);
      launch(KGatherState{sy, ctx->sl, ctx->d_q0, ctx->d_p0}, (long)sy.B * sy.Q, 8);
    }
  }
  for (int i = 0; i < n_inner; ++i) {
    const bool last = i == n_inner - 1;
    for (int h = 0; h < nh; ++h) {
      enter(h);
      if (i > 0) {
        launch_rows(KFlow{sy, ctx->sl, ctx->w, 0, 0, 0, 1.0}, sy.Q, sy.B, 8);
      } else if (ctx->mom_tangent) {
        if (pending_kick) launch_rows(KKick2FlowPg{sy, ctx->sl, ctx->w, kick}, sy.Q, sy.B, 8);
        else launch_rows(KKickFlowPg{sy, ctx->sl, ctx->w, kick}, sy.Q, sy.B, 8);
      } else {
        launch(KKick{sy, ctx->sl, ctx->w, 0, 1, kick}, (long)sy.B * sy.Q, 8);
        project_momentum(ctx, 0, 3, 2);
        launch_rows(KFlow{sy, ctx->sl, ctx->w, 0, 0, 1, 1.0}, sy.Q, sy.B, 8);
      }
    }
    run_projection(ctx, newton, 0, 0, ctol, ptol, dtol, max_iters, two ? &full : nullptr, 0);
    for (int h = 0; h < nh; ++h) {
      enter(h);
      state_eval_core(ctx, 1, last, 3);
      const bool fix_in_jw = last && ctx->plan.mom_fix_in_jp;
      if (fix_in_jw)
        launch_rows(KMomFixEdges{KMomFixInitPg{sy, ctx->sl, ctx->w, 1}}, sy.U + sy.V0 + (sy.Q - sy.U - sy.NV), sy.B, 8);
      else
        launch_rows(KMomFixInitPg{sy, ctx->sl, ctx->w, 1}, sy.Q, sy.B, 8);
      const bool flow_in_update = last && ctx->plan.rev_flow_in_update;
      if (last)
        project_momentum_and_kick_direction(ctx, 1, false, fix_in_jw, flow_in_update);
      else
        project_momentum(ctx, 1, 0, 0);
      launch_rows(KFlow{sy, ctx->sl, ctx->w, 1, 1, 0, -1.0}, flow_in_update ? sy.U : sy.Q, sy.B, 8);
    }
    run_projection(ctx, newton, 1, 1, ctol, ptol, dtol, max_iters, two ? &full : nullptr, 1);
    for (int h = 0; h < nh; ++h) {
      enter(h);
      launch_colmax(KRevDiff{sy, ctx->sl, ctx->w}, (sy.Q + 1) / 2, sy.B, 8);
      launch(KRevCheck{ctx->w, rev_tol}, sy.B);
      if (last) {
        if (!skip_end_kick) launch_rows(KKickPg{sy, ctx->sl, ctx->w, 1, 0, kick}, sy.Q, sy.B, 8);
        launch(KCommit{ctx->sl, ctx->w}, sy.B);
      } else {
        launch(KCommitInner{ctx->sl, ctx->w, ctx->d_ncommit}, sy.B);
      }
    }
  }
  if (two) {
    restore_view(ctx, full);
    streams_join();
    const int extra = n_inner;
    ctx->counters[0] -= extra, ctx->counters[1] -= extra, ctx->counters[3] -= extra, ctx->counters[4] -= 1;
  }
  return 0;
}
static void step_finish(chmc_ctx* ctx, bool masked, int n_inner, int* status, int* iters_fwd, int* iters_bwd,
                        double* rev_err) {
  const Sys& sy = ctx->sy;
  bool any_failed = false;
  {
    const size_t nb = (size_t)sy.B * (sizeof(double) + 3 * sizeof(int));
    ctx->h_out.resize(nb);
    d2h(ctx->h_out.data(), ctx->d_out, nb);
    const unsigned char* h = ctx->h_out.data();
    if (rev_err) memcpy(rev_err, h, sizeof(double) * sy.B);
    h += sizeof(double) * sy.B;
    if (status) memcpy(status, h, sizeof(int) * sy.B);
    if (iters_fwd) memcpy(iters_fwd, h + sizeof(int) * sy.B, sizeof(int) * sy.B);
    if (iters_bwd) memcpy(iters_bwd, h + 2 * sizeof(int) * sy.B, sizeof(int) * sy.B);
    const int* st = reinterpret_cast<const int*>(h);
    for (int c = 0; c < sy.B; ++c) any_failed = any_failed || st[c] > 0;
    if (n_inner > 1 && any_failed) {
      std::vector<int> nc(sy.B), mask(sy.B);
      d2h(nc.data(), ctx->d_ncommit, sizeof(int) * sy.B);
      bool any = false;
      for (int c = 0; c < sy.B; ++c) any = (mask[c] = st[c] > 0 && nc[c] > 0) || any;
      if (any) {
        h2d(ctx->d_act, mask.data(), sizeof(int) * sy.B);
        ctx->last_active_null = true;
        ctx->last_active.clear();
        launch(KInnerRestore{sy, ctx->sl, ctx->d_q0, ctx->d_p0, ctx->d_act}, (long)sy.B * sy.Q, 8);
        launch(KBegin{ctx->w, ctx->d_act, nullptr, 1.0}, sy.B);
        state_eval(ctx, 0);
        h2d(ctx->w.status, st, sizeof(int) * sy.B);
      }
    }
  }
  ctx->counters[5]++;
  ctx->mom_tangent = ctx->mom_tangent || (!masked && !any_failed);
}
extern "C" int chmc_leapfrog_step(chmc_ctx* ctx, const double* dt, const int* active, int n_inner, int newton,
                                  double ctol, double ptol, double dtol, int max_iters, double rev_tol, int* status,
                                  int* iters_fwd, int* iters_bwd, double* rev_err) {
  CHMC_ENTER("chmc_leapfrog_step")
  if (!dt) return fail("chmc_leapfrog_step: dt is required");
  if (n_inner < 1) return fail("chmc_leapfrog_step: n_inner_step must be at least 1");
  if (step_enqueue(ctx, dt, active, nullptr, n_inner, newton, ctol, ptol, dtol, max_iters, rev_tol)) return -1;
  step_finish(ctx, active != nullptr, n_inner, status, iters_fwd, iters_bwd, rev_err);
  CHMC_LEAVE("chmc_leapfrog_step")
}

extern "C" int chmc_leapfrog_steps(chmc_ctx* ctx, const double* dt, const int* active, const int* n_steps, int n_steps_all,
                                   int n_inner, int newton, double ctol, double ptol, double dtol, int max_iters,
                                   double rev_tol, int* n_done, int* status, int* iters_fwd, int* iters_bwd, double* rev_err) {
  CHMC_ENTER("chmc_leapfrog_steps")
  if (!dt) return fail("chmc_leapfrog_steps: dt is required");
  if (n_inner < 1) return fail("chmc_leapfrog_steps: n_inner_step must be at least 1");
  if (!n_steps && n_steps_all < 0) return fail("chmc_leapfrog_steps: negative number of steps");
  const Sys& sy = ctx->sy;
  const int B = sy.B;
#ifdef CHMC_WAVE_KERNELS
  if (traj_waves(ctx, n_inner, newton)) {
    int longest = n_steps_all;
    if (n_steps) {
      longest = 0;
      for (int c = 0; c < B; ++c) longest = n_steps[c] > longest ? n_steps[c] : longest;
    }
    if (step_enqueue(ctx, dt, active, nullptr, n_inner, newton, ctol, ptol, dtol, max_iters, rev_tol, n_steps,
                     n_steps ? longest : n_steps_all, true))
      return -1;
    std::vector<int> nd(B), st(B);
    d2h(nd.data(), ctx->d_ndone, sizeof(int) * B);
    step_finish(ctx, active != nullptr, 1, st.data(), iters_fwd, iters_bwd, rev_err);
    long long tot = 0;
    for (int c = 0; c < B; ++c) {
      if (st[c] < 0) nd[c] = 0;
      tot += nd[c] + (st[c] > 0);
    }
    if (n_done) memcpy(n_done, nd.data(), sizeof(int) * B);
    if (status) memcpy(status, st.data(), sizeof(int) * B);
    ctx->counters[5] += longest > 0 ? longest - 1 : 0;
    (void)tot;
    CHMC_LEAVE("chmc_leapfrog_steps")
  }
#endif
  std::vector<int> act(B), left(B), nd(B, 0), st_out(B, 0), itf(B, 0), itb(B, 0), st(B), f(B), b(B);
  std::vector<double> rv(B, 0.0), r1(B);
  int longest = 0;
  for (int c = 0; c < B; ++c) {
    act[c] = active ? (active[c] != 0) : 1;
    left[c] = act[c] ? (n_steps ? n_steps[c] : n_steps_all) : 0;
    if (left[c] < 0) left[c] = 0;
    st_out[c] = act[c] ? 0 : -1;
    longest = left[c] > longest ? left[c] : longest;
  }
  const bool fuse_kicks = !n_steps && n_inner == 1 && !sy.m0;
  bool pending = false;
  for (int k = 0; k < longest; ++k) {
    std::vector<int> run(B);
    bool any = false;
    for (int c = 0; c < B; ++c) any = (run[c] = act[c] && left[c] > 0) || any;
    if (!any) break;
    const bool skip = fuse_kicks && ctx->mom_tangent && k + 1 < longest;
    if (step_enqueue(ctx, dt, run.data(), nullptr, n_inner, newton, ctol, ptol, dtol, max_iters, rev_tol, nullptr, 1, false, skip,
                     pending))
      return -1;
    pending = skip;
    step_finish(ctx, true, n_inner, st.data(), f.data(), b.data(), r1.data());
    for (int c = 0; c < B; ++c) {
      if (!run[c]) continue;
      itf[c] += f[c], itb[c] += b[c];
      if (st[c] == 0 || st[c] == 3) rv[c] = r1[c];
      if (st[c] == 0) {
        nd[c] += 1, left[c] -= 1;
      } else {
        st_out[c] = st[c], left[c] = 0;
      }
    }
  }
  if (n_done) memcpy(n_done, nd.data(), sizeof(int) * B);
  if (status) memcpy(status, st_out.data(), sizeof(int) * B);
  if (iters_fwd) memcpy(iters_fwd, itf.data(), sizeof(int) * B);
  if (iters_bwd) memcpy(iters_bwd, itb.data(), sizeof(int) * B);
  if (rev_err) memcpy(rev_err, rv.data(), sizeof(double) * B);
  CHMC_LEAVE("chmc_leapfrog_steps")
}

static void tree_alloc(chmc_ctx* ctx) {
  if (ctx->have_tree) return;
  const int B = ctx->sy.B;
  TreeState& t = ctx->tree;
  t.h0 = alloc<double>(ctx, B), t.sub_logw = alloc<double>(ctx, B), t.sum_acc = alloc<double>(ctx, B), t.u = alloc<double>(ctx, B);
  t.alive = alloc<int>(ctx, B), t.run = alloc<int>(ctx, B), t.take = alloc<int>(ctx, B), t.n_step = alloc<int>(ctx, B);
  t.failed = alloc<int>(ctx, B), t.diverged = alloc<int>(ctx, B), t.n_running = alloc<int>(ctx, 1);
  t.logw = alloc<double>(ctx, B), t.u2 = alloc<double>(ctx, B);
  t.fwd = alloc<int>(ctx, B), t.at_pos = alloc<int>(ctx, B), t.at_neg = alloc<int>(ctx, B), t.moved = alloc<int>(ctx, B);
  t.depth = alloc<int>(ctx, B), t.done = alloc<int>(ctx, B), t.acc = alloc<int>(ctx, B), t.need = alloc<int>(ctx, B);
  t.counts = alloc<int>(ctx, 2);
  if (!ctx->d_tree_part) {
    const int ng = rowsum_groups(ctx->sy.Q);
    ctx->d_tree_part = alloc<double>(ctx, (size_t)B * ng * CHMC_ROWSUM_MAX);
    ctx->d_tree_out = alloc<double>(ctx, (size_t)B * CHMC_ROWSUM_MAX);
    ctx->d_tree_mask = alloc<int>(ctx, 2 * (size_t)B);
  }
  ctx->have_tree = true;
}
static void hamiltonian_enqueue(chmc_ctx* ctx) {
  const Sys& sy = ctx->sy;
  launch_rowsum(KNormRow{sy, ctx->sl}, sy.Q, sy.B, 2, ctx->w.part, 8);
  launch(KHamiltonian{sy, ctx->sl, ctx->w, ctx->npart_sum, ctx->d_ham}, sy.B);
}
extern "C" int chmc_tree_begin(chmc_ctx* ctx, double* h0) {
  CHMC_ENTER("chmc_tree_begin")
  tree_alloc(ctx);
  hamiltonian_enqueue(ctx);
  launch(KTreeBegin{ctx->tree, ctx->d_ham}, ctx->sy.B);
  if (h0) d2h(h0, ctx->tree.h0, sizeof(double) * ctx->sy.B);
  CHMC_LEAVE("chmc_tree_begin")
}
extern "C" int chmc_tree_subtree(chmc_ctx* ctx) {
  CHMC_ENTER("chmc_tree_subtree")
  if (!ctx->have_tree) return fail("chmc_tree_subtree: chmc_tree_begin has not been called");
  launch(KTreeSubBegin{ctx->tree}, ctx->sy.B);
  CHMC_LEAVE("chmc_tree_subtree")
}
extern "C" int chmc_tree_step(chmc_ctx* ctx, const double* dt, int n_inner, int newton, double ctol, double ptol,
                              double dtol, int max_iters, double rev_tol, const double* u_leaf, double max_delta_h,
                              void* sub_prop_q_dev, void* sub_sum_dev, void* ck_p_dev, void* ck_sum_dev, void* ck_end_dev,
                              int store_slot, int check_lo, int n_check, int* n_running) {
  CHMC_ENTER("chmc_tree_step")
  if (!ctx->have_tree) return fail("chmc_tree_step: chmc_tree_begin has not been called");
  if (!dt || !u_leaf || !sub_prop_q_dev || !sub_sum_dev || !ck_p_dev || !ck_sum_dev || !n_running)
    return fail("chmc_tree_step: null argument");
  if (n_inner < 1) return fail("chmc_tree_step: n_inner_step must be at least 1");
  if (n_check < 0 || n_check > CHMC_TREE_MAXCHK || check_lo < 0 || store_slot < -1)
    return fail("chmc_tree_step: checkpoint range out of bounds");
  const Sys& sy = ctx->sy;
  TreeState& t = ctx->tree;
  h2d(t.u, u_leaf, sizeof(double) * sy.B);
  if (step_enqueue(ctx, dt, nullptr, t.run, n_inner, newton, ctol, ptol, dtol, max_iters, rev_tol)) return -1;
  hamiltonian_enqueue(ctx);
  launch(KTreeDecide{t, ctx->w.status, ctx->d_ham, max_delta_h}, sy.B);
  const int ng = rowsum_groups(sy.Q), nacc = 6 * n_check;
  launch_rowsum(KTreeLeaf{sy, ctx->sl, t.run, t.take, (double*)sub_prop_q_dev, (double*)sub_sum_dev, (double*)ck_p_dev,
                          (double*)ck_sum_dev, (double*)ck_end_dev, store_slot, check_lo, n_check},
                sy.Q, sy.B, nacc, ctx->d_tree_part, 8);
  if (nacc) {
    launch(KTreeLeafFinish{sy, ctx->sl, t.run, ctx->d_tree_part, ng, nacc, ctx->d_tree_out, (double*)ck_end_dev, check_lo},
           sy.B);
    launch(KTreeTurn{t, ctx->d_tree_out, nacc}, sy.B);
  }
  launch(KTreeCount{t, sy.B}, 1);
  step_finish(ctx, true, n_inner, nullptr, nullptr, nullptr, nullptr);
  d2h(n_running, t.n_running, sizeof(int));
  CHMC_LEAVE("chmc_tree_step")
}
extern "C" int chmc_tree_doubling_begin(chmc_ctx* ctx, const double* u_dir, const void* neg_q_dev, const void* neg_p_dev,
                                        const void* pos_q_dev, const void* pos_p_dev, void* sub_sum_dev, int* n_alive) {
  CHMC_ENTER("chmc_tree_doubling_begin")
  if (!ctx->have_tree) return fail("chmc_tree_doubling_begin: chmc_tree_begin has not been called");
  if (!u_dir || !neg_q_dev || !neg_p_dev || !pos_q_dev || !pos_p_dev || !sub_sum_dev || !n_alive)
    return fail("chmc_tree_doubling_begin: null argument");
  const Sys& sy = ctx->sy;
  TreeState& t = ctx->tree;
  h2d(t.u2, u_dir, sizeof(double) * sy.B);
  dev_zero(t.counts, sizeof(int) * 2);
  launch(KTreeDoubleBegin{t}, sy.B);
  dev_zero(sub_sum_dev, sizeof(double) * (size_t)sy.B * sy.Q);
  int cnt[2] = {0, 0};
  d2h(cnt, t.counts, sizeof(cnt));
  *n_alive = cnt[0];
  if (cnt[1] > 0) {
    launch(KTreeRestoreEdge{sy, ctx->sl, t, (const double*)neg_q_dev, (const double*)neg_p_dev, (const double*)pos_q_dev,
                            (const double*)pos_p_dev}, (long)sy.B * sy.Q, 8);
    ctx->last_active_null = true;
    ctx->last_active.clear();
    begin_all(ctx, nullptr, t.need);
    state_eval(ctx, 0);
  }
  CHMC_LEAVE("chmc_tree_doubling_begin")
}
extern "C" int chmc_tree_doubling_end(chmc_ctx* ctx, const double* u_accept, int depth, void* prop_q_dev,
                                      const void* sub_prop_q_dev, void* sum_mom_dev, const void* sub_sum_dev, void* neg_q_dev,
                                      void* neg_p_dev, void* pos_q_dev, void* pos_p_dev, int* n_alive) {
  CHMC_ENTER("chmc_tree_doubling_end")
  if (!ctx->have_tree) return fail("chmc_tree_doubling_end: chmc_tree_begin has not been called");
  if (!u_accept || !prop_q_dev || !sub_prop_q_dev || !sum_mom_dev || !sub_sum_dev || !neg_q_dev || !neg_p_dev ||
      !pos_q_dev || !pos_p_dev || !n_alive)
    return fail("chmc_tree_doubling_end: null argument");
  const Sys& sy = ctx->sy;
  TreeState& t = ctx->tree;
  h2d(t.u2, u_accept, sizeof(double) * sy.B);
  launch(KTreeDoubleDecide{t, depth}, sy.B);
  const int ng = rowsum_groups(sy.Q);
  launch_rowsum(KTreeDoubleRows{sy, ctx->sl, t, (double*)prop_q_dev, (double*)sum_mom_dev, (double*)neg_q_dev,
                                (double*)neg_p_dev, (double*)pos_q_dev, (double*)pos_p_dev, (const double*)sub_prop_q_dev,
                                (const double*)sub_sum_dev},
                sy.Q, sy.B, 2, ctx->d_tree_part, 8);
  dev_zero(t.counts, sizeof(int) * 2);
  launch(KTreeDoubleFinish{t, ctx->d_tree_part, ng}, sy.B);
  int cnt[2] = {0, 0};
  d2h(cnt, t.counts, sizeof(cnt));
  *n_alive = cnt[0];
  CHMC_LEAVE("chmc_tree_doubling_end")
}
extern "C" int chmc_tree_get_doubling(chmc_ctx* ctx, int* moved, int* depth, double* logw) {
  CHMC_ENTER("chmc_tree_get_doubling")
  if (!ctx->have_tree) return fail("chmc_tree_get_doubling: chmc_tree_begin has not been called");
  const TreeState& t = ctx->tree;
  if (moved) d2h(moved, t.moved, sizeof(int) * ctx->sy.B);
  if (depth) d2h(depth, t.depth, sizeof(int) * ctx->sy.B);
  if (logw) d2h(logw, t.logw, sizeof(double) * ctx->sy.B);
  CHMC_LEAVE("chmc_tree_get_doubling")
}
extern "C" int chmc_tree_get(chmc_ctx* ctx, int* alive, int* run, int* n_step, int* failed, int* diverged, double* sub_logw,
                             double* sum_acc) {
  CHMC_ENTER("chmc_tree_get")
  if (!ctx->have_tree) return fail("chmc_tree_get: chmc_tree_begin has not been called");
// ... 115 lines not shown
```

### manifold_mcmc_for_diffusions_amd/csrc/chmc_core.h

```cpp
#pragma once
#include <math.h>
#include <stdint.h>
#include "chmc_model.h"

#define CHMC_FI __attribute__((always_inline))
#if defined(__HIPCC__)
#define CHMC_UNROLL _Pragma("unroll")
#define CHMC_UNROLL4 _Pragma("unroll 4")
#else
#define CHMC_UNROLL
#define CHMC_UNROLL4
#endif

namespace chmc {

#ifndef CHMC_FWD_DEPTH
#define CHMC_FWD_DEPTH 4
#endif
#define CHMC_Q_PAD 256
#define CHMC_TPAD 16

struct BlockDesc {
  int obs0, nobs, first, last;
  int row0, nrows, ny;
// ... 1339 lines not shown
  }
  CHMC_HD unsigned long long operator()(int c, int idx) const {
    int which = this->which, qsel = this->qsel;
    if (TGT == 0) newton_select(w, c, which, qsel);
    const int s = sl.cur[c] ^ which;
    const int col = idx * VEC;
    const size_t qi = (size_t)c * sy.Q + sy.U + col;
    double* tgt = TGT == 0 ? (qsel ? w.qb : pick(sl.q, s ^ 1))
                           : TGT == 1 ? (psel == 0 ? pick(sl.p, s) : psel == 1 ? w.pb : psel == 3 ? pick(sl.pg, s) : pick(sl.p, s ^ 1))
                           : TGT == 3 ? pick(sl.p, s) : w.pb;
    double d[VEC], old[VEC], d2[VEC], old2[VEC];
    double* tgt2 = TGT == 3 ? pick(sl.p, s) : nullptr;
    if (TGT == 3) tgt = pick(sl.pg, s);
    if (TGT != 2) {
      if (VEC == 2) {
        const double2_ o = *reinterpret_cast<const double2_*>(tgt + qi);
        old[0] = o.x, old[VEC - 1] = o.y;
      } else {
        old[0] = tgt[qi];
      }
    }
    if (TGT == 3) {
      if (VEC == 2) {
        const double2_ o = *reinterpret_cast<const double2_*>(tgt2 + qi);
        old2[0] = o.x, old2[VEC - 1] = o.y;
      } else {
        old2[0] = tgt2[qi];
      }
    }
    if (col < sy.NV) {
      const int g = col < sy.V0 ? 0 : (col - sy.V0) / sy.V / sy.S;
      const int b = sy.obs2blk[g];
      const double* lam = w.lampad + ((size_t)c * sy.Kmax + b) * RM;
      const double* lam2 = w.lampad2 + ((size_t)c * sy.Kmax + b) * RM;
      const double* Jv = pick(sl.Jv, s) + (size_t)c * RM * sy.NV + col;
      CHMC_UNROLL
      for (int k = 0; k < VEC; ++k) d[k] = 0.0, d2[k] = 0.0;
      const int m = col < sy.V0 ? 0 : g - sy.blk[b].obs0;
      const int nr = sy.blk[b].nrows;
      CHMC_UNROLL
      for (int i = 0; i < RM; ++i) {
        if (i >= m && i < nr) {
          if (VEC == 2) {
            const double2_ jv = ld2_stream(Jv + (size_t)i * sy.NV);
            d[0] += jv.x * lam[i];
            d[VEC - 1] += jv.y * lam[i];
            if (TGT == 3) d2[0] += jv.x * lam2[i], d2[VEC - 1] += jv.y * lam2[i];
          } else {
            const double jv = Jv[(size_t)i * sy.NV];
            d[0] += jv * lam[i];
            if (TGT == 3) d2[0] += jv * lam2[i];
          }
        }
      }
    } else {
      CHMC_UNROLL
      for (int k = 0; k < VEC; ++k) {
        d[k] = ncol_part(c, col + k, which);
        if (TGT == 3) d2[k] = ncol_part2(c, col + k, which);
      }
    }
    unsigned long long r = 0ULL;
    CHMC_UNROLL
    for (int k = 0; k < VEC; ++k) {
      if (TGT == 0) {
        const unsigned long long vb = absbits(d[k]);
        r = vb > r ? vb : r;
      }
      old[k] = TGT == 2 ? d[k] : old[k] - d[k];
      if (TGT == 3) old2[k] -= d2[k];
    }
    if (VEC == 2) {
      double2_ o;
      o.x = old[0], o.y = old[VEC - 1];
      *reinterpret_cast<double2_*>(tgt + qi) = o;
      if (TGT == 3) {
        o.x = old2[0], o.y = old2[VEC - 1];
        *reinterpret_cast<double2_*>(tgt2 + qi) = o;
      }
    } else {
      tgt[qi] = old[0];
      if (TGT == 3) tgt2[qi] = old2[0];
    }
    return r;
  }
};

template <int RM, int X, int V>
struct KRowsFromPB {
  Sys sy;
  Slots sl;
  CHMC_HD void operator()(int tid) const {
    const int TS = sy.T * sy.S;
    const int c = tid / TS, st = tid - c * TS;
    const int s = sl.cur[c];
    const int g = st / sy.S;
    const int b = sy.obs2blk[g];
    const int m = g - sy.blk[b].obs0;
    const double* lf = pick(sl.LF, s) + ((((size_t)c * sy.Kmax + b) * sy.NOBS + m) * RM) * X;
    const double* pb = pick(sl.PB, s) + ((size_t)c * TS + st) * (X * V);
    double* Jv = pick(sl.Jv, s) + (size_t)c * RM * sy.NV + sy.V0 + (size_t)st * V;
    double pbv[X * V];
    CHMC_UNROLL
    for (int k = 0; k < X * V; ++k) pbv[k] = pb[k];
    for (int i = 0; i < RM; ++i)
      CHMC_UNROLL
      for (int d = 0; d < V; ++d) {
        double t = 0.0;
        CHMC_UNROLL
        for (int a = 0; a < X; ++a) t += lf[i * X + a] * pbv[a * V + d];
        Jv[(size_t)i * sy.NV + d] = t;
      }
  }
};
template <int RM, int X, int TGT>
struct KMuF {
  Sys sy;
  Slots sl;
  Work w;
  int which;
  CHMC_FI CHMC_HD void operator()(int tid) const {
    const int a = tid % X;
    int r = tid / X;
    const int m = r % sy.NOBS;
    r /= sy.NOBS;
    const int b = r % sy.K, c = r / sy.K;
    int which = this->which, qsel_unused = 0;
    if (TGT == 0 ? !newton_select(w, c, which, qsel_unused) : !w.ok[c]) return;
    const size_t cb = (size_t)c * sy.Kmax + b;
    double t = 0.0, t2 = 0.0;
    if (m < sy.blk[b].nobs) {
      const double* lam = w.lampad + cb * RM;
      const double* lam2 = w.lampad2 + cb * RM;
      const double* lf = pick(sl.LF, sl.cur[c] ^ which) + (cb * sy.NOBS + m) * RM * X;
      const int nr = sy.blk[b].nrows;
      for (int i = 0; i < RM; ++i)
        if (i < nr) {
          t += lam[i] * lf[i * X + a];
          if (TGT == 3) t2 += lam2[i] * lf[i * X + a];
        }
    }
    w.muF[(cb * sy.NOBS + m) * X + a] = t;
    if (TGT == 3) w.muF2[(cb * sy.NOBS + m) * X + a] = t2;
  }
};
template <int RM, int X, int V, int TGT, int NS = 1>
struct KUpdatePB {
  static constexpr bool kFinish = false;
  Sys sy;
  Slots sl;
  Work w;
  int which, qsel, psel;
  int flow_rev = 0;
  CHMC_HD void rev_flow2(int c, int s, size_t i, double px, double py) const {
    const double2_ q0 = ld2_stream(pick(sl.q, s) + i);
    const double dt = -1.0 * w.dt[c];
    double2_ qn;
    qn.x = q0.x + dt * px, qn.y = q0.y + dt * py;
    stv2(w.qb + i, qn, true, true);
  }
  CHMC_HD void rev_flow1(int c, int s, size_t i, double px) const {
    const double dt = -1.0 * w.dt[c];
    w.qb[i] = pick(sl.q, s)[i] + dt * px;
  }
  CHMC_HD bool active(int c) const {
    int p_ = 0, q_ = 0;
    return TGT == 0 ? newton_select(w, c, p_, q_) : w.ok[c] != 0;
  }
  CHMC_HD unsigned long long* red(int c) const { return TGT == 0 ? &w.ndq[c] : nullptr; }
  CHMC_FI CHMC_HD unsigned long long operator()(int c, int idx) const {
    int which = this->which, qsel = this->qsel;
    if (TGT == 0) newton_select(w, c, which, qsel);
    const int s = sl.cur[c] ^ which;
    const size_t off = (size_t)c * sy.Q + sy.U;
    double* tgt = (TGT == 0 ? (qsel ? w.qb : pick(sl.q, s ^ 1))
                            : TGT == 1 ? (psel == 0 ? pick(sl.p, s) : psel == 1 ? w.pb : psel == 3 ? pick(sl.pg, s) : pick(sl.p, s ^ 1))
                                       : pick(sl.pg, s)) + off;
    double* tgt2 = TGT == 3 ? pick(sl.p, s) + off : nullptr;
    const int TS = sy.T * sy.S;
    unsigned long long r = 0ULL;
    if (idx < TS / NS) {
      const int st0 = idx * NS;
      const int g = st0 / sy.S;
      const int b = sy.obs2blk[g];
      const int m = g - sy.blk[b].obs0;
      const size_t mo = (((size_t)c * sy.Kmax + b) * sy.NOBS + m) * X;
      const double* pb = pick(sl.PB, s) + ((size_t)c * TS + st0) * (X * V);
      const size_t to = sy.V0 + (size_t)st0 * V;
      const bool wide = V == 2 && !((sy.Q | sy.U | sy.V0) & 1);
      double old[NS * V], old2[NS * V], pbv[NS * X * V], mu[X], mu2[X];
      CHMC_UNROLL
      for (int e = 0; e < NS; ++e) {
        if (wide) {
          const double2_ o = *reinterpret_cast<const double2_*>(tgt + to + e * V);
          old[e * V] = o.x, old[e * V + V - 1] = o.y;
          if (TGT == 3) {
            const double2_ o2 = *reinterpret_cast<const double2_*>(tgt2 + to + e * V);
            old2[e * V] = o2.x, old2[e * V + V - 1] = o2.y;
          }
        } else {
          CHMC_UNROLL
          for (int k = 0; k < V; ++k) {
            old[e * V + k] = tgt[to + e * V + k];
            if (TGT == 3) old2[e * V + k] = tgt2[to + e * V + k];
          }
        }
      }
      if ((NS * X * V) % 2 == 0) {
        CHMC_UNROLL
        for (int k = 0; k < NS * X * V; k += 2) {
          const double2_ v = ld2_stream(pb + k);
          pbv[k] = v.x, pbv[k + 1 < NS * X * V ? k + 1 : k] = v.y;
        }
      } else {
        CHMC_UNROLL
        for (int k = 0; k < NS * X * V; ++k) pbv[k] = pb[k];
      }
      CHMC_UNROLL
      for (int a = 0; a < X; ++a) {
        mu[a] = w.muF[mo + a];
        if (TGT == 3) mu2[a] = w.muF2[mo + a];
      }
      CHMC_UNROLL
      for (int e = 0; e < NS; ++e)
        CHMC_UNROLL
        for (int k = 0; k < V; ++k) {
          double tt = 0.0, t2 = 0.0;
          CHMC_UNROLL
          for (int a = 0; a < X; ++a) {
            tt += mu[a] * pbv[e * X * V + a * V + k];
            if (TGT == 3) t2 += mu2[a] * pbv[e * X * V + a * V + k];
          }
          if (TGT == 0) {
            const unsigned long long vb = absbits(tt);
            r = vb > r ? vb : r;
          }
          old[e * V + k] -= tt;
          if (TGT == 3) old2[e * V + k] -= t2;
        }
      CHMC_UNROLL
      for (int e = 0; e < NS; ++e) {
        if (wide) {
          double2_ o;
          o.x = old[e * V], o.y = old[e * V + V - 1];
          *reinterpret_cast<double2_*>(tgt + to + e * V) = o;
          if (TGT == 3) {
            o.x = old2[e * V], o.y = old2[e * V + V - 1];
            *reinterpret_cast<double2_*>(tgt2 + to + e * V) = o;
            if (flow_rev) rev_flow2(c, s, off + to + e * V, o.x, o.y);
          }
        } else {
          CHMC_UNROLL
          for (int k = 0; k < V; ++k) {
            tgt[to + e * V + k] = old[e * V + k];
            if (TGT == 3) {
              tgt2[to + e * V + k] = old2[e * V + k];
              if (flow_rev) rev_flow1(c, s, off + to + e * V + k, old2[e * V + k]);
            }
          }
        }
      }
    } else {
      const int e = idx - TS / NS;
      double d = 0.0, d2 = 0.0;
      int col;
      if (e < sy.V0) {
        col = e;
        const int b = sy.obs2blk[0];
        const double* lam = w.lampad + ((size_t)c * sy.Kmax + b) * RM;
        const double* lam2 = w.lampad2 + ((size_t)c * sy.Kmax + b) * RM;
        const double* Jv = pick(sl.Jv, s) + (size_t)c * RM * sy.NV + col;
        const int nr = sy.blk[b].nrows;
        for (int i = 0; i < RM; ++i)
          if (i < nr) {
            const double jv = Jv[(size_t)i * sy.NV];
            d += jv * lam[i];
            if (TGT == 3) d2 += jv * lam2[i];
          }
      } else {
        const int t = e - sy.V0;
        col = sy.NV + t;
        const int b = sy.obs2blk[t];
        const int j = t - sy.blk[b].obs0;
        if (j < sy.blk[b].ny) {
          const double sg = sigma_at(sy, pick(sl.q, s) + (size_t)c * sy.Q);
          d = sg * w.lampad[((size_t)c * sy.Kmax + b) * RM + j];
          if (TGT == 3) d2 = sg * w.lampad2[((size_t)c * sy.Kmax + b) * RM + j];
        }
      }
      if (TGT == 0) r = absbits(d);
      tgt[col] -= d;
      if (TGT == 3) {
        const double pn = tgt2[col] - d2;
        tgt2[col] = pn;
        if (flow_rev) rev_flow1(c, s, off + col, pn);
      }
    }
    return r;
  }
};

template <class M>
struct KInitInterp {
  Sys sy;
  double* q;
  const double* u;
  const double* v0;
  const double* xobs;
  CHMC_HD void operator()(int tid) const {
    constexpr int X = M::X, V = M::V;
    static_assert(X == V, "the interpolation solve needs a square noise matrix");
    const int TS = sy.T * sy.S;
    const int c = tid / TS, s = tid - c * TS;
    const int t = s / sy.S, i = s - t * sy.S;
    double* qc = q + (size_t)c * sy.Q;
    const double* uc = u + (size_t)c * sy.U;
    ChainConsts<M> cc;
    cc.init(uc, sy.dl);
    double xa[X], xs[X], dlt[X], f0[X], zero[V], A[X * X], Bm[X * V], rhs[X];
    if (t == 0) {
      M::gx0(cc.z, v0 + (size_t)c * sy.V0, xa);
    } else {
      for (int a = 0; a < X; ++a) xa[a] = xobs[((size_t)c * sy.T + t - 1) * X + a];
    }
    for (int a = 0; a < X; ++a) {
      dlt[a] = (xobs[((size_t)c * sy.T + t) * X + a] - xa[a]) / sy.S;
      xs[a] = xa[a] + i * dlt[a];
    }
    for (int a = 0; a < V; ++a) zero[a] = 0.0;
    M::step(cc.k, xs, zero, f0);
    M::jac_ab(cc.k, xs, zero, A, Bm);
    for (int a = 0; a < X; ++a) rhs[a] = dlt[a] - (f0[a] - xs[a]);
    int piv[X];
    lu_factor<X>(Bm, piv);
    lu_solve<X, 1>(Bm, piv, rhs);
    double* vq = qc + sy.U + sy.V0 + (size_t)s * V;
    for (int a = 0; a < V; ++a) vq[a] = rhs[a];
    if (s == 0) {
      for (int a = 0; a < sy.U; ++a) qc[a] = uc[a];
      for (int a = 0; a < sy.V0; ++a) qc[sy.U + a] = v0[(size_t)c * sy.V0 + a];
      if (sy.noisy)
        for (int a = 0; a < sy.T; ++a) qc[sy.U + sy.NV + a] = 0.0;
    }
  }
};

CHMC_HD inline void philox4x32_10(uint32_t c0, uint32_t c1, uint32_t c2, uint32_t c3, uint32_t k0, uint32_t k1,
                                  uint32_t* out) {
  for (int r = 0; r < 10; ++r) {
    const uint64_t p0 = (uint64_t)0xD2511F53u * c0, p1 = (uint64_t)0xCD9E8D57u * c2;
    const uint32_t n0 = (uint32_t)(p1 >> 32) ^ c1 ^ k0, n1 = (uint32_t)p1;
    const uint32_t n2 = (uint32_t)(p0 >> 32) ^ c3 ^ k1, n3 = (uint32_t)p0;
    c0 = n0, c1 = n1, c2 = n2, c3 = n3;
    k0 += 0x9E3779B9u, k1 += 0xBB67AE85u;
  }
  out[0] = c0, out[1] = c1, out[2] = c2, out[3] = c3;
}
struct KNormalFill {
  Sys sy;
  Slots sl;
  unsigned long long seed, draw;
  int chain_offset;
  CHMC_HD void operator()(int tid) const {
    const int npair = (sy.Q + 1) / 2;
    const int c = tid / npair, j = tid - c * npair;
    uint32_t r[4];
    philox4x32_10((uint32_t)j, (uint32_t)draw, (uint32_t)(c + chain_offset), (uint32_t)(draw >> 32), (uint32_t)seed,
                  (uint32_t)(seed >> 32), r);
    const double u1 = (((uint64_t)r[0] << 21) ^ ((uint64_t)r[1] >> 11)) * (1.0 / 9007199254740992.0) +
                      (0.5 / 9007199254740992.0);
    const double u2 = (((uint64_t)r[2] << 21) ^ ((uint64_t)r[3] >> 11)) * (1.0 / 9007199254740992.0);
    const double rad = sqrt(-2.0 * log(u1)), ang = 6.283185307179586476925286766559 * u2;
    double* p = pick(sl.p, sl.cur[c]) + (size_t)c * sy.Q;
    p[2 * j] = rad * cos(ang);
    if (2 * j + 1 < sy.Q) p[2 * j + 1] = rad * sin(ang);
  }
};

struct KCheck {
  Work w;
  double ctol, ptol, dtol;
  int max_iters, B;
  int* iters_dst;
  int slot;
  CHMC_HD void operator()(int c) const {
    if (c == 0) w.n_active[(slot + 1) & 3] = 0;
    if (!w.nw[c]) return;
    if (w.nw[c] != 1) {
      atomic_add_i32(w.n_active + slot, 1);
      return;
    }
    const int i = ++w.iters[c];
    const double err = w.err[c], ndq = bitsd(w.ndq[c]);
    const bool diverged = (err > dtol) || (err != err);
    const bool converged = (err < ctol) && (ndq < ptol);
    if (i >= max_iters || diverged || converged) {
      w.nw[c] = 0;
      int st = converged ? 0 : (diverged ? 2 : 1);
      w.nstat[c] = st;
      if (st) w.ok[c] = 0, w.status[c] = st;
      if (iters_dst) iters_dst[c] += i;
    } else {
      atomic_add_i32(w.n_active + slot, 1);
    }
  }
};

struct KNewtonBegin {
  Work w;
  CHMC_HD void operator()(int c) const {
    w.nw[c] = w.ok[c];
    w.iters[c] = 0;
    w.err[c] = -1.0;
    w.ndq[c] = 0x7ff0000000000000ULL;
    w.nstat[c] = 0;
    if (c == 0) w.n_active[0] = 0;
  }
};

struct KNewtonEnd {
  Work w;
  int* iters_dst;
  CHMC_HD void operator()(int c) const {
    if (!w.nw[c]) return;
    w.nw[c] = 0;
    w.nstat[c] = 1;
    w.ok[c] = 0, w.status[c] = 1;
    if (iters_dst) iters_dst[c] += w.iters[c];
  }
};

template <int RM>
struct KJw {
  Sys sy;
  Slots sl;
  Work w;
  int which, vsel_;
  CHMC_HD void operator()(int tid) const {
    const int i = tid % RM;
    const int cbk = tid / RM;
    const int c = cbk / sy.K;
    const int b = cbk - c * sy.K;
    if (!w.ok[c]) return;
    const BlockDesc bd = sy.blk[b];
    const int s = sl.cur[c] ^ which;
    const bool minv = (vsel_ & 256) != 0;
    const int vsel = vsel_ & 255;
    const double* vct = (vsel == 0 ? pick(sl.p, s) : vsel == 1 ? w.pb : vsel == 2 ? w.vin : vsel == 4 ? pick(sl.pg, s) : pick(sl.p, s ^ 1)) + (size_t)c * sy.Q;
// ... 40 lines not shown
    const int s = sl.cur[c] ^ which;
    pick(sl.pg, s)[tid] = pick(sl.grad, s)[tid] + (sy.gaussian ? 0.0 : pick(sl.q, s)[tid]);
  }
};
struct KKickPg {
  Sys sy;
  Slots sl;
  Work w;
  int which, out_other;
  double hfrac;
  CHMC_HD bool active(int c) const { return w.ok[c] != 0; }
  CHMC_FI CHMC_HD void operator()(int c, int col) const {
    const int s = sl.cur[c] ^ which;
    const double h = hfrac * w.dt[c];
    const size_t i = (size_t)c * sy.Q + col;
    const bool two = col + 1 < sy.Q, wide = two && !(sy.Q & 1);
    const double2_ p0 = ldv2(pick(sl.p, s) + i, wide, two), g = ldv2(pick(sl.pg, s) + i, wide, two);
    double2_ o;
    o.x = p0.x - h * g.x, o.y = p0.y - h * g.y;
    stv2((out_other ? pick(sl.p, s ^ 1) : pick(sl.p, s)) + i, o, wide, two);
  }
};
struct KFlow {
  Sys sy;
  Slots sl;
  Work w;
  int from, dst, from_p_other;
  double sign;
  CHMC_HD bool active(int c) const { return w.ok[c] != 0; }
  CHMC_FI CHMC_HD void operator()(int c, int col) const {
    const int s = sl.cur[c] ^ from;
    const double dt = sign * w.dt[c];
    const size_t i = (size_t)c * sy.Q + col;
    const bool two = col + 1 < sy.Q, wide = two && !(sy.Q & 1);
    const double2_ q0 = ldv2(pick(sl.q, s) + i, wide, two);
    const double2_ p0 = ldv2((from_p_other ? pick(sl.p, s ^ 1) : pick(sl.p, s)) + i, wide, two);
    double2_ qn, pn;
    if (sy.gaussian) {
      const double sn = sign * w.sdt[c], cs = w.cdt[c];
      qn.x = q0.x * cs + sn * p0.x, qn.y = q0.y * cs + sn * p0.y;
      pn.x = p0.x * cs - sn * q0.x, pn.y = p0.y * cs - sn * q0.y;
    } else {
      qn.x = q0.x + dt * p0.x, qn.y = q0.y + dt * p0.y;
      pn = p0;
    }
    if (sy.m0 && col < sy.U) {
      const double* pu = (from_p_other ? pick(sl.p, s ^ 1) : pick(sl.p, s)) + (size_t)c * sy.Q;
      qn.x = q0.x + dt * metric_inv_u(sy, pu, col);
      if (col + 1 < sy.U) qn.y = q0.y + dt * metric_inv_u(sy, pu, col + 1);
    }
    if (dst == 0) {
      stv2(pick(sl.q, s ^ 1) + i, qn, wide, two);
      if (sy.gaussian || !from_p_other) stv2(pick(sl.p, s ^ 1) + i, pn, wide, two);
    } else {
      stv2(w.qb + i, qn, wide, two);
    }
  }
};
struct KMomFixInitPg {
  Sys sy;
  Slots sl;
  Work w;
  int which;
  CHMC_HD bool active(int c) const { return w.ok[c] != 0; }
  CHMC_FI CHMC_HD void operator()(int c, int col) const {
    const int s = sl.cur[c] ^ which;
    const size_t i = (size_t)c * sy.Q + col;
    const bool two = col + 1 < sy.Q, wide = two && !(sy.Q & 1);
    const double2_ qp = ldv2(pick(sl.q, s ^ 1) + i, wide, two), qn = ldv2(pick(sl.q, s) + i, wide, two);
    const double2_ pn = ldv2(pick(sl.p, s) + i, wide, two), gr = ldv2(pick(sl.grad, s) + i, wide, two);
    double sc;
    double2_ flow, po, go;
    if (sy.gaussian) {
      sc = w.cdt[c] / w.sdt[c];
      flow.x = (qp.x + w.sdt[c] * pn.x) / w.cdt[c], flow.y = (qp.y + w.sdt[c] * pn.y) / w.cdt[c];
    } else {
      sc = 1.0 / w.dt[c];
      flow.x = qp.x + w.dt[c] * pn.x, flow.y = qp.y + w.dt[c] * pn.y;
    }
    po.x = pn.x - sc * (flow.x - qn.x), po.y = pn.y - sc * (flow.y - qn.y);
    go.x = gr.x + (sy.gaussian ? 0.0 : qn.x), go.y = gr.y + (sy.gaussian ? 0.0 : qn.y);
    if (sy.m0 && col < sy.U) {
      if (col != 0) {
        if (col + 1 >= sy.U && two) {
          pick(sl.p, s)[i + 1] = po.y;
          pick(sl.pg, s)[i + 1] = go.y;
        }
        return;
      }
      const size_t cq = (size_t)c * sy.Q;
      const double* qpu = pick(sl.q, s ^ 1) + cq;
      const double* qnu = pick(sl.q, s) + cq;
      double* pu = pick(sl.p, s) + cq;
      double mv[8], pnew[8];
      for (int a = 0; a < sy.U; ++a) mv[a] = qpu[a] + w.dt[c] * metric_inv_u(sy, pu, a) - qnu[a];
      for (int a = 0; a < sy.U; ++a) pnew[a] = pu[a] - sc * metric_mul_u(sy, mv, a);
      for (int a = 0; a < sy.U; ++a) {
        pu[a] = pnew[a];
        pick(sl.pg, s)[cq + a] = pick(sl.grad, s)[cq + a] + qnu[a];
      }
      return;
    }
    stv2(pick(sl.p, s) + i, po, wide, two);
    stv2(pick(sl.pg, s) + i, go, wide, two);
  }
};
struct KMomFixEdges {
  KMomFixInitPg f;
  CHMC_HD bool active(int c) const { return f.active(c); }
  CHMC_FI CHMC_HD void operator()(int c, int col) const {
    const int head = f.sy.U + f.sy.V0;
    f(c, col < head ? col : col - head + f.sy.U + f.sy.NV);
  }
};
struct KKickFlowPg {
  Sys sy;
  Slots sl;
  Work w;
  double hfrac;
  CHMC_HD bool active(int c) const { return w.ok[c] != 0; }
  CHMC_FI CHMC_HD void operator()(int c, int col) const {
    const int s = sl.cur[c];
    const double h = hfrac * w.dt[c];
    const size_t i = (size_t)c * sy.Q + col;
    const bool two = col + 1 < sy.Q, wide = two && !(sy.Q & 1);
    const double2_ q0 = ldv2(pick(sl.q, s) + i, wide, two), pp = ldv2(pick(sl.p, s) + i, wide, two);
    const double2_ g = ldv2(pick(sl.pg, s) + i, wide, two);
    double2_ p0, qn, pn;
    p0.x = pp.x - h * g.x, p0.y = pp.y - h * g.y;
    if (sy.gaussian) {
      const double sn = w.sdt[c], cs = w.cdt[c];
      qn.x = q0.x * cs + sn * p0.x, qn.y = q0.y * cs + sn * p0.y;
      pn.x = p0.x * cs - sn * q0.x, pn.y = p0.y * cs - sn * q0.y;
    } else {
      qn.x = q0.x + w.dt[c] * p0.x, qn.y = q0.y + w.dt[c] * p0.y;
      pn = p0;
    }
    if (sy.m0 && col < sy.U) {
      const double* pu = pick(sl.p, s) + (size_t)c * sy.Q;
      const double* gu = pick(sl.pg, s) + (size_t)c * sy.Q;
      double t0 = 0.0, t1 = 0.0;
      for (int b = 0; b < sy.U; ++b) {
        const double pb = pu[b] - h * gu[b];
        t0 += sy.m0[sy.U * sy.U + col * sy.U + b] * pb;
        if (col + 1 < sy.U) t1 += sy.m0[sy.U * sy.U + (col + 1) * sy.U + b] * pb;
      }
      qn.x = q0.x + w.dt[c] * t0;
      if (col + 1 < sy.U) qn.y = q0.y + w.dt[c] * t1;
    }
    stv2(pick(sl.q, s ^ 1) + i, qn, wide, two);
    stv2(pick(sl.p, s ^ 1) + i, pn, wide, two);
  }
};
struct KKick2FlowPg {
  Sys sy;
  Slots sl;
  Work w;
  double hfrac;
  CHMC_HD bool active(int c) const { return w.ok[c] != 0; }
  CHMC_FI CHMC_HD void operator()(int c, int col) const {
    const int s = sl.cur[c];
    const double h = hfrac * w.dt[c];
    const size_t i = (size_t)c * sy.Q + col;
    const bool two = col + 1 < sy.Q, wide = two && !(sy.Q & 1);
    const double2_ q0 = ldv2(pick(sl.q, s) + i, wide, two), pp = ldv2(pick(sl.p, s) + i, wide, two);
    const double2_ g = ldv2(pick(sl.pg, s) + i, wide, two);
    double2_ p1, p0, qn, pn;
    p1.x = pp.x - h * g.x, p1.y = pp.y - h * g.y;
    p0.x = p1.x - h * g.x, p0.y = p1.y - h * g.y;
    if (sy.gaussian) {
      const double sn = w.sdt[c], cs = w.cdt[c];
      qn.x = q0.x * cs + sn * p0.x, qn.y = q0.y * cs + sn * p0.y;
      pn.x = p0.x * cs - sn * q0.x, pn.y = p0.y * cs - sn * q0.y;
    } else {
      qn.x = q0.x + w.dt[c] * p0.x, qn.y = q0.y + w.dt[c] * p0.y;
      pn = p0;
    }
    stv2(pick(sl.p, s) + i, p1, wide, two);
    stv2(pick(sl.q, s ^ 1) + i, qn, wide, two);
    stv2(pick(sl.p, s ^ 1) + i, pn, wide, two);
  }
};
struct KRevDiff {
  static constexpr bool kFinish = false;
  Sys sy;
  Slots sl;
  Work w;
  CHMC_HD bool active(int c) const { return w.ok[c] != 0; }
  CHMC_HD unsigned long long* red(int c) const { return &w.rev[c]; }
  CHMC_FI CHMC_HD unsigned long long operator()(int c, int idx) const {
    const int col = 2 * idx;
    const size_t i = (size_t)c * sy.Q + col;
    const double* qs = pick(sl.q, sl.cur[c]);
    if (col + 1 < sy.Q && (sy.Q & 1) == 0) {
      const double2_ a = *reinterpret_cast<const double2_*>(w.qb + i), b = *reinterpret_cast<const double2_*>(qs + i);
      const unsigned long long u = absbits(a.x - b.x), v = absbits(a.y - b.y);
      return u > v ? u : v;
    }
    unsigned long long r = absbits(w.qb[i] - qs[i]);
    if (col + 1 < sy.Q) {
      const unsigned long long v = absbits(w.qb[i + 1] - qs[i + 1]);
      r = v > r ? v : r;
    }
    return r;
  }
};
struct KRevCheck {
  Work w;
  double tol;
  CHMC_FI CHMC_HD void operator()(int c) const {
    if (!w.ok[c]) return;
    const double r = bitsd(w.rev[c]);
    if (!(r <= tol)) w.ok[c] = 0, w.status[c] = 3;
  }
};
struct KCommit {
  Slots sl;
  Work w;
  CHMC_FI CHMC_HD void operator()(int c) const {
    if (w.ok[c]) sl.cur[c] ^= 1;
  }
};
struct KBegin {
  Work w;
  const int* active;
  const double* dt;
  double scale;
  CHMC_HD void operator()(int c) const {
    w.ok[c] = active ? (active[c] != 0) : 1;
    w.status[c] = w.ok[c] ? 0 : -1;
    if (dt) {
      const double h = scale * dt[c];
      w.dt[c] = h;
      w.sdt[c] = sin(h);
      w.cdt[c] = cos(h);
    }
    w.rev[c] = 0ULL;
  }
};
struct KAddIters {
  Work w;
  int* dst;
  CHMC_HD void operator()(int c) const {
    if (w.ok[c] || w.status[c] > 0) dst[c] += w.iters[c];
  }
};
struct KCommitInner {
  Slots sl;
  Work w;
  int* ncommit;
  CHMC_HD void operator()(int c) const {
    if (w.ok[c]) {
      sl.cur[c] ^= 1;
      ncommit[c] += 1;
      w.rev[c] = 0ULL;
    }
  }
};
struct KCopyPadMasked {
  Work w;
  double* dst;
  const double* src;
  int n;
  CHMC_HD void operator()(int tid) const {
    if (w.ok[tid / n]) dst[tid] = src[tid];
  }
};

#define CHMC_TREE_MAXCHK 10
#define CHMC_ROWSUM_MAX (6 * CHMC_TREE_MAXCHK)
struct KTreeLeaf {
  Sys sy;
  Slots sl;
  const int* run;
  const int* take;
  double* sub_prop_q;
  double* sub_sum;
  double* ck_p;
  double* ck_sum;
  double* ck_end;
  int store, lo, nchk;
  CHMC_HD bool active(int c) const { return run[c] != 0; }
  CHMC_HD double2_ vel(const double* base, size_t cq, int col, double2_ p) const {
    if (sy.m0 && col < sy.U) {
      p.x = metric_inv_u(sy, base + cq, col);
      if (col + 1 < sy.U) p.y = metric_inv_u(sy, base + cq, col + 1);
    }
    return p;
  }
  CHMC_HD void operator()(int c, int col, double* acc) const {
    const int s = sl.cur[c];
    const size_t cq = (size_t)c * sy.Q, i = cq + col, BQ = (size_t)sy.B * sy.Q;
    const bool two = col + 1 < sy.Q, wide = two && !(sy.Q & 1);
    const double2_ q = ldv2(pick(sl.q, s) + i, wide, two), p = ldv2(pick(sl.p, s) + i, wide, two);
    double2_ S = ldv2(sub_sum + i, wide, two);
    S.x += p.x, S.y += p.y;
    stv2(sub_sum + i, S, wide, two);
    if (take[c]) stv2(sub_prop_q + i, q, wide, two);
    if (store >= 0) {
      stv2(ck_p + store * BQ + i, p, wide, two);
      stv2(ck_sum + store * BQ + i, S, wide, two);
    }
    const double2_ vp = vel(pick(sl.p, s), cq, col, p);
    double2_ a_r, cs_r;
    a_r.x = a_r.y = cs_r.x = cs_r.y = 0.0;
    CHMC_UNROLL
    for (int kk = 0; kk < CHMC_TREE_MAXCHK; ++kk) {
      const int k = nchk - 1 - kk;
      if (k >= 0) {
        const double* cp = ck_p + (size_t)(lo + k) * BQ;
        const double2_ a = ldv2(cp + i, wide, two), cs = ldv2(ck_sum + (size_t)(lo + k) * BQ + i, wide, two);
        const double2_ va = vel(cp, cq, col, a);
        const double sx = S.x - cs.x + a.x, sy_ = two ? S.y - cs.y + a.y : 0.0;
        acc[6 * k] += va.x * sx + (two ? va.y * sy_ : 0.0);
        acc[6 * k + 1] += vp.x * sx + (two ? vp.y * sy_ : 0.0);
        if (ck_end && kk > 0) {
          const double* ce = ck_end + (size_t)(lo + k) * BQ;
          const double* cr = ck_p + (size_t)(lo + k + 1) * BQ;
          const double2_ pm = ldv2(ce + i, wide, two);
          const double2_ vm = vel(ce, cq, col, pm), vr = vel(cr, cq, col, a_r);
          const double r1x = cs_r.x - cs.x + a.x, r1y = two ? cs_r.y - cs.y + a.y : 0.0;
          const double r2x = S.x - cs_r.x + a_r.x + pm.x, r2y = two ? S.y - cs_r.y + a_r.y + pm.y : 0.0;
          acc[6 * k + 2] += va.x * r1x + (two ? va.y * r1y : 0.0);
          acc[6 * k + 3] += vr.x * r1x + (two ? vr.y * r1y : 0.0);
          acc[6 * k + 4] += vm.x * r2x + (two ? vm.y * r2y : 0.0);
          acc[6 * k + 5] += vp.x * r2x + (two ? vp.y * r2y : 0.0);
        }
        a_r = a, cs_r = cs;
      }
    }
    if (ck_end && nchk > 0) {
      double* ce = ck_end + (size_t)lo * BQ + i;
      if (col >= sy.U) stv2(ce, p, wide, two);
// ... 298 lines not shown
```

### manifold_mcmc_for_diffusions_amd/csrc/chmc_plan.h

```cpp
#pragma once
#include <climits>
#include <cstdlib>

#ifndef CHMC_RETRACT_WAVES
#define CHMC_RETRACT_WAVES 8
#endif
#ifndef CHMC_CHAIN_SCAN_WAVES
#define CHMC_CHAIN_SCAN_WAVES 4
#endif
#ifndef CHMC_CHAIN_WG4_MAX_PER_CU
#define CHMC_CHAIN_WG4_MAX_PER_CU 4
#endif

namespace chmc {

constexpr int kSwitchUnset = INT_MIN;
struct Switches {
  bool compact_rows = true, gram_mfma = false;
  int par_scan = kSwitchUnset, par_waves = kSwitchUnset, row_split = 0, halves = 1;
  bool no_fwd_scan = false, step_fusions = true;
  int retract_kernel = kSwitchUnset;
};
inline Switches read_switches() {
  auto env = [](const char* name, int unset) {
    const char* e = getenv(name);
    return e ? atoi(e) : unset;
  };
  static const bool compact_rows = env("CHMC_COMPACT_ROWS", 1) != 0, gram_mfma = env("CHMC_GRAM_MFMA", 0) != 0;
  Switches s;
  s.compact_rows = compact_rows, s.gram_mfma = gram_mfma;
  s.par_scan = env("CHMC_PAR_SCAN", kSwitchUnset), s.par_waves = env("CHMC_PAR_WAVES", kSwitchUnset);
  s.row_split = env("CHMC_ROW_SPLIT", 0), s.halves = env("CHMC_HALVES", 1);
  s.no_fwd_scan = getenv("CHMC_NO_FWD_SCAN") != nullptr, s.step_fusions = env("CHMC_STEP_FUSIONS", 1) != 0;
  s.retract_kernel = env("CHMC_RETRACT_KERNEL", kSwitchUnset);
  return s;
}

struct PlanInput {
  int rmt;
  int num_partition;
  int K[2];
  int longest;
  int chain_steps;
  bool s_tiles8;
  int V;
  bool even_dims;
  bool gaussian;
  bool wave_kernels;
  Switches sw;
  Switches call;
};

enum RowFamily { RowsCompact, RowsStored, RowsStoredMfma };
enum FwdScan { FwdPar , FwdWave , FwdFunctor  };
enum StateSweep {
  StateLean,
  StateIvlComb,
  StateIvlCombWg,
  StateLdsrowsGram,
  StateLdsrowsGramMfma,
  StateRevWave,
  StateRevStoreGramMfma
};
enum NewtonSweep {
  NewtonIvlFsm,
  NewtonIvlComb,
  NewtonRevWave,
  NewtonRevStoreGramMfma,
  Newton16IvlCombWg,
  Newton16IvlCombFactor,
  Newton16IvlComb,
  Newton16LdsrowsGram,
  Newton16LdsrowsGramMfma
};
enum GldSweep {
  GldQxLean,
  GldIvl,
  GldCompactFwdStored,
  GldStored
};
enum JpPass { JpPb , JpPbWg , JpWave  };

struct PartitionPlan {
  StateSweep state;
  NewtonSweep newton;
  GldSweep gld;
  JpPass jp;
  bool rebuild_rows;
  bool retract_chain;
  bool traj_chain;
};
struct KernelPlan {
  RowFamily rows;
  bool pb_allocated;
  bool par_scan;
  FwdScan fwd;
  FwdScan fwd_cold;
  int fwd_waves;
  FwdScan nld;
  int nld_waves;
  bool mom_fix_in_jp;
  bool rev_flow_in_update;
  int retract_kernel;
  PartitionPlan part[2];
};

inline int par_waves_for(int env, long longest) {
  if (env == 1 || env == 2 || env == 4) return env;
  return longest >= 4096 ? 4 : longest >= 2048 ? 2 : 1;
}
inline bool few_long_blocks(int nblocks_per_chain, long longest) { return nblocks_per_chain <= 4 && longest >= 1024; }

inline KernelPlan make_plan(const PlanInput& in) {
  const Switches& sw = in.sw;
  KernelPlan pl{};
  const bool rows16 = in.rmt > 8;
  const int kmax = in.K[0] > in.K[in.num_partition - 1] ? in.K[0] : in.K[in.num_partition - 1];
  const bool chain16_layout = kmax == 1 && rows16;

  const bool compact = in.wave_kernels && sw.compact_rows && !sw.gram_mfma;
  pl.rows = compact ? RowsCompact : sw.gram_mfma ? RowsStoredMfma : RowsStored;
  pl.pb_allocated = compact || (in.wave_kernels && sw.compact_rows && rows16);

  pl.par_scan = sw.par_scan != kSwitchUnset ? sw.par_scan != 0
                                            : few_long_blocks(kmax, in.longest) || (chain16_layout && sw.compact_rows && !sw.gram_mfma);
  pl.fwd_waves = chain16_layout && sw.par_waves == kSwitchUnset ? CHMC_CHAIN_SCAN_WAVES : par_waves_for(sw.par_waves, in.longest);
  pl.fwd_cold = in.wave_kernels && in.s_tiles8 && !in.call.no_fwd_scan ? FwdWave : FwdFunctor;
  pl.fwd = in.wave_kernels && pl.par_scan ? FwdPar : pl.fwd_cold;
  const bool nld_par = in.call.par_scan != kSwitchUnset ? in.call.par_scan != 0 : few_long_blocks(1, in.chain_steps);
  pl.nld = nld_par ? FwdPar : in.s_tiles8 ? FwdWave : FwdFunctor;
  pl.nld_waves = par_waves_for(in.call.par_waves, in.chain_steps);

  const bool step_fusions = pl.pb_allocated && in.call.step_fusions && !rows16;
  pl.mom_fix_in_jp = step_fusions && in.V == 2 && in.even_dims;
  pl.rev_flow_in_update = step_fusions && !in.gaussian;
  pl.retract_kernel = in.call.retract_kernel;

  for (int p = 0; p < in.num_partition; ++p) {
    PartitionPlan& pp = pl.part[p];
    const int K = in.K[p];
    const bool split = sw.row_split == 1 ? false : (sw.row_split == 2 || sw.row_split == 4) ? true : K <= 4;
    const bool ivl16 = rows16 && compact && split;
    const bool chain16 = chain16_layout && ivl16;
    if (rows16) {
      pp.state = chain16 ? StateIvlCombWg : ivl16 ? StateIvlComb : sw.gram_mfma ? StateLdsrowsGramMfma : StateLdsrowsGram;
      pp.newton = chain16 ? Newton16IvlCombWg
                  : compact ? (K == 1 ? Newton16IvlCombFactor : Newton16IvlComb)
                  : sw.gram_mfma ? Newton16LdsrowsGramMfma : Newton16LdsrowsGram;
      pp.gld = ivl16 ? GldIvl : compact ? GldCompactFwdStored : GldStored;
    } else {
      pp.state = compact ? StateLean : sw.gram_mfma ? StateRevStoreGramMfma : StateRevWave;
      pp.newton = compact ? (K <= 64 ? NewtonIvlFsm : NewtonIvlComb) : sw.gram_mfma ? NewtonRevStoreGramMfma : NewtonRevWave;
      pp.gld = compact ? GldQxLean : GldStored;
    }
    pp.jp = chain16 ? JpPbWg : compact ? JpPb : JpWave;
    pp.rebuild_rows = compact && (!rows16 || ivl16);
    pp.retract_chain = compact && rows16 && K == 1;
    pp.traj_chain = pp.retract_chain && ivl16;
  }
  return pl;
}

inline int chain_kernel_waves(const KernelPlan& pl, bool eligible, int B, int num_cus, bool newton, bool half_batches) {
  if (!eligible || !newton || half_batches) return 0;
  const int want = pl.retract_kernel != kSwitchUnset ? pl.retract_kernel
                   : B <= num_cus ? 1 : B <= CHMC_CHAIN_WG4_MAX_PER_CU * num_cus ? 2 : 0;
  return want == 1 ? CHMC_RETRACT_WAVES : want == 2 ? 4 : 0;
}

}
```

### manifold_mcmc_for_diffusions_amd/csrc/chmc_wave.h

```cpp
#pragma once
#include <type_traits>
#include "chmc_core.h"

namespace chmc {

#ifdef CHMC_PLAIN_STREAM
__device__ inline double ld_stream(const double* p) { return *p; }
#else
__device__ inline double ld_stream(const double* p) { return __builtin_nontemporal_load(p); }
#endif

__device__ __forceinline__ void st_async(double* p, double v) {
  asm volatile("global_store_dwordx2 %0, %1, off\n\ts_nop 1" : : "v"(p), "v"(v) : "memory");
}
__device__ __forceinline__ void st_async2(double* p, double v0, double v1) {
  typedef double d2v __attribute__((ext_vector_type(2)));
  const d2v v = {v0, v1};
  asm volatile("global_store_dwordx4 %0, %1, off\n\ts_nop 1" : : "v"(p), "v"(v) : "memory");
}

__device__ inline double bcast0(double x) {
  union { double d; int i[2]; } u;
  u.d = x;
  u.i[0] = __builtin_amdgcn_readfirstlane(u.i[0]);
// ... 4256 lines not shown
  const int c = blockIdx.x;
  if (c >= sy.B) return;
  const int s_ = sl.cur[c];
  const int S = sy.S, L = sy.T * sy.S;
  const double* q = pick(sl.q, s_) + (size_t)c * sy.Q;
  const double* trj = pick(sl.traj, s_) + (size_t)c * sy.TRJ;
  const double* vbase = q + sy.U + sy.V0;
  double* out = xobs_out + (size_t)c * sy.T * X;
  ChainConsts<M> cc;
  cc.init(q, sy.dl);
  double x0[X];
  M::gx0(cc.z, q + sy.U, x0);
  const int m = (L + 63) >> 6;
  const int s0 = lane * m, s1 = (s0 + m < L ? s0 + m : L);
  const bool have = s0 < L;
  double Ul[X];
  {
    const int b0 = have ? sy.obs2blk[s0 / S] : 0;
#pragma unroll
    for (int a = 0; a < X; ++a) Ul[a] = lane == 0 ? x0[a] : (have ? trj[(size_t)(s0 + CHMC_TPAD * b0) * X + a] : 0.0);
  }
  bool converged = false;
  for (int sweep = 0; sweep < MAXS && !converged; ++sweep) {
    double x[X], P[X * X];
#pragma unroll
    for (int a = 0; a < X; ++a) x[a] = Ul[a];
#pragma unroll
    for (int i = 0; i < X * X; ++i) P[i] = (i / X == i % X) ? 1.0 : 0.0;
    constexpr int CH = 8;
    double vb[2][CH * V];
    auto fetch = [&](int base, double* dst) {
#pragma unroll
      for (int j = 0; j < CH; ++j) {
        int sj = base + j;
        sj = sj < L ? sj : L - 1;
#pragma unroll
        for (int a = 0; a < V; ++a) dst[j * V + a] = vbase[(size_t)sj * V + a];
      }
    };
    auto run = [&](int base, const double* src) {
#pragma unroll
      for (int j = 0; j < CH; ++j) {
        const int s = base + j;
        if (s < s1) {
          double vv[V], A[X * X], Bm[X * V], xn[X], Pn[X * X];
#pragma unroll
          for (int a = 0; a < V; ++a) vv[a] = src[j * V + a];
          M::jac_ab(cc.k, x, vv, A, Bm);
          M::step(cc.k, x, vv, xn);
          matmul_xx<X>(A, P, Pn);
#pragma unroll
          for (int i = 0; i < X * X; ++i) P[i] = Pn[i];
#pragma unroll
          for (int a = 0; a < X; ++a) x[a] = xn[a];
          if ((s + 1) % S == 0) {
            const int t = (s + 1) / S - 1;
#pragma unroll
            for (int a = 0; a < X; ++a) out[t * X + a] = x[a];
          }
        }
      }
    };
    if (have) fetch(s0, vb[0]);
    for (int base = s0; base < s1; base += 2 * CH) {
      fetch(base + CH, vb[1]);
      run(base, vb[0]);
      fetch(base + 2 * CH, vb[0]);
      run(base + CH, vb[1]);
    }
    double ec[X], Pc[X * X], Unext[X];
#pragma unroll
    for (int a = 0; a < X; ++a) Unext[a] = __shfl_down(Ul[a], 1, 64);
    const bool junction = have && s1 < L;
#pragma unroll
    for (int a = 0; a < X; ++a) ec[a] = junction ? x[a] - Unext[a] : 0.0;
#pragma unroll
    for (int i = 0; i < X * X; ++i) Pc[i] = junction ? P[i] : ((i / X == i % X) ? 1.0 : 0.0);
#pragma unroll
    for (int o = 1; o < 64; o <<= 1) {
      double Pp[X * X], ep[X], Pn[X * X];
#pragma unroll
      for (int i = 0; i < X * X; ++i) Pp[i] = __shfl_up(Pc[i], o, 64);
#pragma unroll
      for (int a = 0; a < X; ++a) ep[a] = __shfl_up(ec[a], o, 64);
      if (lane >= o) {
#pragma unroll
        for (int a = 0; a < X; ++a) {
          double tt = ec[a];
#pragma unroll
          for (int d = 0; d < X; ++d) tt += Pc[a * X + d] * ep[d];
          ec[a] = tt;
        }
        matmul_xx<X>(Pc, Pp, Pn);
#pragma unroll
        for (int i = 0; i < X * X; ++i) Pc[i] = Pn[i];
      }
    }
    double dl[X], Un[X];
#pragma unroll
    for (int a = 0; a < X; ++a) {
      const double up = __shfl_up(ec[a], 1, 64);
      dl[a] = lane == 0 ? 0.0 : up;
    }
    bool still = true;
#pragma unroll
    for (int a = 0; a < X; ++a) still = still && dl[a] == 0.0;
#pragma unroll
    for (int a = 0; a < X; ++a) {
      double tt = 0.0;
#pragma unroll
      for (int d = 0; d < X; ++d) tt += P[a * X + d] * dl[d];
      Un[a] = still ? x[a] : x[a] + tt;
    }
    int unsettled = 0;
#pragma unroll
    for (int a = 0; a < X; ++a) {
      const double nu = __shfl_up(Un[a], 1, 64);
      if (lane > 0 && have) {
        const double old = Ul[a];
        const bool same = nu == old || (nu != nu && old != old);
        const bool close = fabs(nu - old) <= 1e-13 * (fabs(nu) > 1.0 ? fabs(nu) : 1.0);
        unsettled |= !(same || close);
        Ul[a] = nu;
      }
    }
    converged = __ballot(unsettled) == 0ULL;
  }
  if (!converged && lane == 0) {
    double x[X], xn[X];
#pragma unroll
    for (int a = 0; a < X; ++a) x[a] = x0[a];
    for (int s = 0; s < L; ++s) {
      M::step(cc.k, x, vbase + (size_t)s * V, xn);
#pragma unroll
      for (int a = 0; a < X; ++a) x[a] = xn[a];
      if ((s + 1) % S == 0) {
        const int t = (s + 1) / S - 1;
#pragma unroll
        for (int a = 0; a < X; ++a) out[t * X + a] = x[a];
      }
    }
  }
}

__device__ __forceinline__ void lds_barrier() { asm volatile("s_waitcnt lgkmcnt(0)\n\ts_barrier" ::: "memory"); }

__device__ inline bool scan_select(const Work& w, int c, int use_nw, int& which, int& qsel) {
  (void)which, (void)qsel;
  return use_nw ? w.nw[c] == 1 : w.ok[c] != 0;
}
#ifndef CHMC_SCAN_HELPERS
#define CHMC_SCAN_HELPERS 1
#endif
template <class M, int RM, bool STORE>
__global__ void __launch_bounds__(STORE ? 64 * (1 + CHMC_SCAN_HELPERS) : 64)
    k_fwd_scan(Sys sy, Slots sl, Work w, int which, int qsel, int use_nw, int store_traj) {
  constexpr int X = M::X, V = M::V, PF = 8;
  constexpr int NLD = PF * V / 2;
  constexpr int NST = PF * X / 2;
  constexpr int TBV = PF * V * 8;
#ifndef CHMC_SCAN_DEPTH
#define CHMC_SCAN_DEPTH (V == 2 ? 4 : 3)
#endif
  constexpr int DEPTH = CHMC_SCAN_DEPTH;
  constexpr int NOUT = (DEPTH - 1) * NLD;
  constexpr int RSD = PF * X + 2;
  static_assert(NOUT <= 63, "vmcnt is a 6-bit field");
#ifndef CHMC_SCAN_NB
#define CHMC_SCAN_NB 1
#endif
  constexpr int NB = CHMC_SCAN_NB;
  __shared__ __attribute__((aligned(16))) double tile[STORE ? 2 : 1][STORE ? NB * 64 * RSD : 2];
  __shared__ double obsv[64 * (2 * RM + 1)];
  const int lane = threadIdx.x & 63;
  const int wave_id = __builtin_amdgcn_readfirstlane(threadIdx.x >> 6);
  const bool helper = STORE && wave_id != 0;
  const int hid = wave_id - 1;
  const int n = sy.B * sy.K, S = sy.S;
  const int tid0 = blockIdx.x * 64;

  int maxL = 0;
  {
    const int t = tid0 + lane;
    int L = 0;
    if (t < n) {
      const int c = t / sy.K;
      int wh_ = which, qs_ = qsel;
      if (scan_select(w, c, use_nw, wh_, qs_)) L = sy.blk[t - c * sy.K].nsteps;
    }
    maxL = L;
#pragma unroll
    for (int off = 32; off > 0; off >>= 1) {
      const int o = __shfl_xor(maxL, off, 64);
      maxL = o > maxL ? o : maxL;
    }
    maxL = __builtin_amdgcn_readfirstlane(maxL);
  }
  if (maxL == 0) return;

  if (helper) {
    double* rp[NST];
    int rL[NST], lo_[NST];
#pragma unroll
    for (int i = 0; i < NST; ++i) {
      const int g = 64 * i + lane, r = g / NST, ch = g - r * NST;
      const int t = tid0 + r;
      rp[i] = w.trajw, rL[i] = 0, lo_[i] = r * RSD + 2 * ch;
      if (t < n) {
        const int c = t / sy.K, b = t - c * sy.K;
        int wh_ = which, qs_ = qsel;
        if (scan_select(w, c, use_nw, wh_, qs_)) {
          const BlockDesc bd = sy.blk[b];
          const int s = sl.cur[c] ^ wh_;
          rp[i] = (store_traj == 2 ? w.trajw : pick(sl.traj, s)) + (size_t)c * sy.TRJ + (size_t)(bd.step0 + CHMC_TPAD * b) * X + 2 * ch;
          rL[i] = bd.nsteps;
        }
      }
    }
#ifdef CHMC_SCAN_PRIO
    __builtin_amdgcn_s_setprio(3);
#endif
    int buf = 0;
    for (int s0 = 0; s0 < maxL; s0 += PF * NB) {
      lds_barrier();
#pragma unroll
      for (int sl_ = 0; sl_ < NB; ++sl_) {
        const int st = s0 + sl_ * PF;
        if (st < maxL) {
          d2_t tt[NST];
#pragma unroll
          for (int i = 0; i < NST; ++i)
            if (i % CHMC_SCAN_HELPERS == hid) tt[i] = *reinterpret_cast<const d2_t*>(&tile[buf][sl_ * 64 * RSD + lo_[i]]);
#pragma unroll
          for (int i = 0; i < NST; ++i)
            if (i % CHMC_SCAN_HELPERS == hid && st < rL[i]) vm_store16_nt(rp[i] + (size_t)st * X, tt[i]);
        }
      }
      buf ^= 1;
    }
    return;
  }

#ifdef CHMC_SCAN_PRIO
  __builtin_amdgcn_s_setprio(3);
#endif
  const int tid = tid0 + lane;
  const int tc = tid < n ? tid : n - 1;
  const int c = tc / sy.K, b = tc - c * sy.K;
  const BlockDesc bd = sy.blk[b];
  const bool act = scan_select(w, c, use_nw, which, qsel) && tid < n;
  const int L = act ? bd.nsteps : 0;
  const int s = sl.cur[c] ^ which;
  const double* q = (qsel ? w.qb : pick(sl.q, s)) + (size_t)c * sy.Q;
  const double* xobs = sy.xobs + (size_t)c * sy.T * X;
  ChainConsts<M> cc;
  cc.init(q, sy.dl);
  const double sig = sy.noisy ? sigma_at(sy, q) : 0.0;
  double x[X], xn[X];
  const double* vb = q + sy.U;
  if (bd.first) {
    M::gx0(cc.z, vb, x);
  } else {
#pragma unroll
    for (int a = 0; a < X; ++a) x[a] = xobs[(bd.obs0 - 1) * X + a];
  }
  double* ov = obsv + lane * (2 * RM + 1);
  {
    const double* nn = q + sy.U + sy.NV;
    for (int j = 0; j < bd.ny; ++j) {
      ov[2 * j] = sy.y[bd.obs0 + j];
      ov[2 * j + 1] = sy.noisy ? nn[bd.obs0 + j] : 0.0;
    }
  }
  double cp[RM];
#pragma unroll
  for (int i = 0; i < RM; ++i) cp[i] = 0.0;

  const char* vp = reinterpret_cast<const char*>(vb + sy.V0 + (size_t)bd.step0 * V);
  d2_t ring[DEPTH][NLD];
#pragma unroll
  for (int d = 0; d < DEPTH; ++d) TileLoad<0, NLD, 0>::run(ring[d], vp + d * TBV);
#pragma unroll
  for (int d = 0; d < DEPTH; ++d) vm_wait<0>(ring[d]);

  int left = S, j = 0;
  for (int s0 = 0; s0 < maxL; s0 += PF * DEPTH) {
#pragma unroll
    for (int d = 0; d < DEPTH; ++d) {
      const int st = s0 + d * PF;
      if (st < maxL) {
        vm_wait<NOUT>(ring[d]);
        if (STORE && st > 0 && (st / PF) % NB == 0) lds_barrier();
        if (st < L) {
          double* lo = STORE ? &tile[((st / PF) / NB) & 1][((st / PF) % NB) * 64 * RSD + lane * RSD] : nullptr;
#pragma unroll
          for (int i = 0; i < PF; ++i) {
            double vt[V];
#pragma unroll
            for (int a = 0; a < V; ++a) vt[a] = ring[d][(i * V + a) >> 1][(i * V + a) & 1];
            if (STORE) {
#pragma unroll
              for (int a = 0; a < X; ++a) lo[i * X + a] = x[a];
            }
            M::step(cc.k, x, vt, xn);
#pragma unroll
            for (int a = 0; a < X; ++a) x[a] = xn[a];
          }
        }
        TileLoad<0, NLD, DEPTH * TBV>::run(ring[d], vp);
        if (st < L) vp += TBV;
        left -= PF;
        if (left == 0) {
          if (st < L && j < bd.ny) {
            const double val = (M::obs(x) + (sy.noisy ? sig * ov[2 * j + 1] : 0.0)) - ov[2 * j];
#pragma unroll
            for (int jj = 0; jj < RM; ++jj)
              if (jj == j) cp[jj] = val;
          }
          ++j;
          left = S;
        }
      }
    }
  }
  if (STORE) lds_barrier();
#pragma unroll
  for (int d = 0; d < DEPTH; ++d) vm_wait<0>(ring[d]);
  if (!act) return;
  if (STORE) {
    double* trow = (store_traj == 2 ? w.trajw : pick(sl.traj, s)) + (size_t)c * sy.TRJ + (size_t)(bd.step0 + CHMC_TPAD * b) * X;
#pragma unroll
    for (int a = 0; a < X; ++a) trow[(size_t)L * X + a] = x[a];
// ... 454 lines not shown
```

Baseline: 51950 steps/s.

## Pair backward retraction with next step's forward retraction in one batched projection

Computes the next leapfrog step's forward position speculatively at the end of the current step's reverse-check flow. It then runs both Newton projections together, with one doubled-grid forward-scan launch serving both work sets. The next step adopts the precomputed projection instead of running its own. The aim is to fill an under-occupied GPU (few workgroups per scan at 256 chains) and halve the serial projection rounds. The cost is an extra Work buffer set, added kernels, and bookkeeping for status and iteration counts.

```diff
diff --git a/manifold_mcmc_for_diffusions_amd/context.py b/manifold_mcmc_for_diffusions_amd/context.py
--- a/manifold_mcmc_for_diffusions_amd/context.py
+++ b/manifold_mcmc_for_diffusions_amd/context.py
@@ -373,7 +373,8 @@
         v = np.array(out[:], dtype=np.int64)
         return dict(par_scan=v[:64], gram_mfma_launches=int(v[64]), gram_valu_launches=int(v[65]),
                     retract_kernel_launches=int(v[66]), traj_kernel_launches=int(v[67]),
-                    newton_fsm_launches=int(v[68]), newton_factor8_launches=int(v[69]), extra=v[68:80])
+                    newton_fsm_launches=int(v[68]), newton_factor8_launches=int(v[69]), pair_scan_rounds=int(v[70]),
+                    newton_scan_launches=int(v[71]), newton_rounds=int(v[72]), extra=v[68:80])
 
     def counters(self):
         out = (C.c_longlong * 8)()
diff --git a/manifold_mcmc_for_diffusions_amd/csrc/chmc_api.inc b/manifold_mcmc_for_diffusions_amd/csrc/chmc_api.inc
--- a/manifold_mcmc_for_diffusions_amd/csrc/chmc_api.inc
+++ b/manifold_mcmc_for_diffusions_amd/csrc/chmc_api.inc
@@ -48,6 +48,10 @@
   PlanInput plan_in{};
   KernelPlan plan{};
   long long diag[16] = {0};
+  Work pw{};
+  int* d_itf_next = nullptr;
+  bool have_pair = false;
+  bool pair_ready = false;
   int round = 0;
   int halves = 1;
   int hB[2] = {0, 0}, hc0[2] = {0, 0};
@@ -246,18 +250,38 @@
     } else if (fwd_ == FwdWave) {                                                                                \
       if (STORE_)                                                                                                \
         launch_blocks(k_fwd_scan<M, RM, true>, ((long)sy.B * sy.K + 63) / 64, 64 * (1 + CHMC_SCAN_HELPERS), 7, sy, c->sl, c->w, WHICH_,   \
-                      QSEL_, USENW_, STORE_);                                                                    \
+                      QSEL_, USENW_, STORE_, c->w, 0, 0);                                                        \
       else                                                                                                       \
         launch_blocks(k_fwd_scan<M, RM, false>, ((long)sy.B * sy.K + 63) / 64, 64, 7, sy, c->sl, c->w, WHICH_,   \
-                      QSEL_, USENW_, STORE_);                                                                    \
+                      QSEL_, USENW_, STORE_, c->w, 0, 0);                                                        \
     } else {                                                                                                     \
       launch(KFwd<M, RM>{sy, c->sl, c->w, WHICH_, QSEL_, USENW_, STORE_}, (long)sy.B * sy.K, 7);                 \
     }                                                                                                            \
     stagger_record();                                                                                            \
   } while (0)
+#define CHMC_FWD_PAIR(W1_, WHICH_, QSEL_, STORE_)                                                                \
+  do {                                                                                                           \
+    const long wg_ = ((long)sy.B * sy.K + 63) / 64;                                                              \
+    if (c->plan.fwd_cold == FwdWave) {                                                                           \
+      if (STORE_)                                                                                                \
+        launch_blocks(k_fwd_scan<M, RM, true, true>, 2 * wg_, 64 * (1 + CHMC_SCAN_HELPERS), 7, sy, c->sl, c->w, WHICH_, QSEL_, 1, \
+                      STORE_, W1_, WHICH_, QSEL_);                                                               \
+      else                                                                                                       \
+        launch_blocks(k_fwd_scan<M, RM, false, true>, 2 * wg_, 64, 7, sy, c->sl, c->w, WHICH_, QSEL_, 1, STORE_, W1_, WHICH_,     \
+                      QSEL_);                                                                                    \
+    } else {                                                                                                     \
+      launch(KFwd<M, RM>{sy, c->sl, c->w, WHICH_, QSEL_, 1, STORE_}, (long)sy.B * sy.K, 7);                      \
+      launch(KFwd<M, RM>{sy, c->sl, W1_, WHICH_, QSEL_, 1, STORE_}, (long)sy.B * sy.K, 7);                       \
+    }                                                                                                            \
+  } while (0)
 #else
 #define CHMC_FWD(WHICH_, QSEL_, USENW_, STORE_, GSEL_) \
   launch(KFwd<M, RM>{sy, c->sl, c->w, WHICH_, QSEL_, USENW_, STORE_}, (long)sy.B * sy.K, 7)
+#define CHMC_FWD_PAIR(W1_, WHICH_, QSEL_, STORE_)                                             \
+  do {            \
+    launch(KFwd<M, RM>{sy, c->sl, c->w, WHICH_, QSEL_, 1, STORE_}, (long)sy.B * sy.K, 7);     \
+    launch(KFwd<M, RM>{sy, c->sl, W1_, WHICH_, QSEL_, 1, STORE_}, (long)sy.B * sy.K, 7);      \
+  } while (0)
 #endif
 
 #define CHMC_UPDATE_PB(TGT_, WHICH_, QSEL_, PSEL_)                                                                \
@@ -539,7 +563,7 @@
   project_momentum(c, which, 4, 3);
 }
 static void project_momentum_and_kick_direction(chmc_ctx* c, int which, bool init_pg, bool fix_in_jw = false,
-                                                bool flow_rev = false) {
+                                                bool flow_rev = false, double* fwd_qb = nullptr, double fwd_hfrac = 0.0) {
   const Sys& sy = c->sy;
   if (init_pg) launch(KInitPg{sy, c->sl, c->w, which}, (long)sy.B * sy.Q, 8);
 #ifdef CHMC_WAVE_KERNELS
@@ -573,7 +597,7 @@
     CHMC_SOLVE_CHAIN(M, RM, 1, 1, sy, c->sl, w2, which, 0, 3);
     if (compact && flow_rev) {
       launch(KMuF<RM, M::X, 3>{sy, c->sl, c->w, which}, (long)sy.B * sy.K * sy.NOBS * M::X, 5);
-      launch_colmax(KUpdatePB<RM, M::X, M::V, 3, 1>{sy, c->sl, c->w, which, 0, 0, 1},
+      launch_colmax(KUpdatePB<RM, M::X, M::V, 3, 1>{sy, c->sl, c->w, which, 0, 0, 1, fwd_qb, fwd_hfrac},
                     sy.T * sy.S + sy.V0 + (sy.noisy ? sy.T : 0), sy.B, 4);
     } else if (compact) {
       CHMC_UPDATE_PB(3, which, 0, 0);
@@ -582,7 +606,7 @@
     }
   });
 #else
-  (void)fix_in_jw, (void)flow_rev;
+  (void)fix_in_jw, (void)flow_rev, (void)fwd_qb, (void)fwd_hfrac;
   project_momentum(c, which, 0, 0);
   project_momentum(c, which, 4, 3);
 #endif
@@ -616,13 +640,36 @@
     if (newton) {
 #ifdef CHMC_WAVE_KERNELS
       CHMC_FWD(prev ^ 1, qsel, use_nw, 2, fwd_guess);
+      c->diag[7]++;
 #else
       (void)fwd_guess, (void)use_nw;
 #endif
     } else {
       CHMC_FWD(prev ^ 1, qsel, use_nw, 0, fwd_guess);
+      c->diag[7]++;
     }
   });
+}
+static void iteration_scan_pair(chmc_ctx* c, int newton, int prev, int qsel, const Work& w1) {
+  const Sys& sy = c->sy;
+  CHMC_DISPATCH(c, {
+    if (newton) {
+#ifdef CHMC_WAVE_KERNELS
+      CHMC_FWD_PAIR(w1, prev ^ 1, qsel, 2);
+      c->diag[7] += c->plan.fwd_cold == FwdWave ? 1 : 2;
+#else
+      (void)w1;
+#endif
+    } else {
+      CHMC_FWD_PAIR(w1, prev ^ 1, qsel, 0);
+#ifdef CHMC_WAVE_KERNELS
+      c->diag[7] += c->plan.fwd_cold == FwdWave ? 1 : 2;
+#else
+      c->diag[7] += 2;
+#endif
+    }
+  });
+  c->diag[6]++;
 }
 static void iteration_after_scan(chmc_ctx* c, int newton, int prev, int qsel) {
   const Sys& sy = c->sy;
@@ -765,6 +812,7 @@
       fwd_guess = it == 0 ? 2 : 1;
       c->round = it;
       iteration(it >= 1 ? 2 * h + (it & 1) : -1);
+      c->diag[8]++;
     }
     c->counters[6]++;
     if (it == 0) continue;
@@ -790,6 +838,96 @@
     enter(h);
     if (sy.B > 0) launch(KNewtonEnd{c->w, count_dir < 0 ? nullptr : (count_dir ? c->d_itb : c->d_itf)}, sy.B);
   }
+  c->round = 0;
+  return 0;
+}
+
+static void pair_alloc(chmc_ctx* c) {
+  if (c->have_pair) return;
+  const Sys& sy = c->sy;
+  const size_t B = sy.B, KM = sy.Kmax, RM = sy.RM, U = sy.U, X = sy.X, Z = sy.Z, ivls = KM * sy.NOBS;
+  Work& w = c->pw;
+  w = c->w;
+  auto zeroed = [&](size_t n) {
+    double* p = alloc<double>(c, n);
+    dev_zero(p, sizeof(double) * n);
+    return p;
+  };
+  w.qb = zeroed(B * sy.Q + CHMC_Q_PAD);
+  w.trajw = alloc<double>(c, B * sy.TRJ);
+  w.cpad = zeroed(B * KM * RM), w.tpad = alloc<double>(c, B * KM * RM), w.lampad = zeroed(B * KM * RM);
+  w.Ew = alloc<double>(c, B * KM * RM * U), w.Cb = alloc<double>(c, B * KM * U * U), w.sb = alloc<double>(c, B * KM * U);
+  w.Dw = alloc<double>(c, B * KM * RM * RM), w.JuL = alloc<double>(c, B * KM * RM * U), w.zbP = alloc<double>(c, B * KM * RM * Z);
+  if (c->plan.pb_allocated) {
+    w.muF = alloc<double>(c, B * ivls * X);
+    w.ivl = alloc<double>(c, B * ivls * (2 * X * X + X * Z));
+  }
+  w.err = alloc<double>(c, B), w.ndq = alloc<unsigned long long>(c, B);
+  w.iters = alloc<int>(c, B), w.nw = alloc<int>(c, B), w.nstat = alloc<int>(c, B), w.ok = alloc<int>(c, B), w.status = alloc<int>(c, B);
+  w.n_active = alloc<int>(c, 4);
+  c->d_itf_next = alloc<int>(c, B);
+  c->have_pair = true;
+}
+
+static int run_projection_pair(chmc_ctx* c, int newton, double ctol, double ptol, double dtol, int max_iters) {
+  const Sys& sy = c->sy;
+  const int prev = 1, qsel = 1;
+  const Work wk[2] = {c->w, c->pw};
+  int* const iters_dst[2] = {c->d_itb, c->d_itf_next};
+  const int dir[2] = {1, 0};
+  auto enter = [&](int p) { c->w = wk[p]; };
+  bool done[2], predict[2], stopped[2] = {false, false};
+  int rounds_done[2] = {0, 0};
+  for (int p = 0; p < 2; ++p) {
+    enter(p);
+    launch(KNewtonBegin{c->w}, sy.B);
+    done[p] = sy.B <= 0;
+    predict[p] = c->proj_stable[dir[p]] >= 3 && c->proj_rounds[dir[p]] >= 2;
+  }
+  for (int it = 0; it < max_iters && !(done[0] && done[1]); ++it) {
+    for (int p = 0; p < 2; ++p)
+      if (!done[p] && predict[p] && it >= c->proj_rounds[dir[p]] && poll_end(2 * p + ((it - 1) & 1)) == 0)
+        done[p] = stopped[p] = true;
+    if (done[0] && done[1]) break;
+    c->round = it;
+    if (!done[0] && !done[1]) {
+      enter(0);
+      iteration_scan_pair(c, newton, prev, qsel, wk[1]);
+    } else {
+      enter(done[0] ? 1 : 0);
+      iteration_scan(c, newton, prev, qsel, it == 0 ? 2 : 1, 1);
+    }
+    for (int p = 0; p < 2; ++p) {
+      if (done[p]) continue;
+      enter(p);
+      iteration_after_scan(c, newton, prev, qsel);
+      const KCheck chk{c->w, ctol, ptol, dtol, max_iters, sy.B, iters_dst[p], it & 3};
+      if (it >= 1) launch_publish(chk, sy.B, c->w.n_active + (it & 3), 2 * p + (it & 1));
+      else launch(chk, sy.B);
+      c->counters[6]++, c->diag[8]++;
+    }
+    if (it == 0) continue;
+    for (int p = 0; p < 2; ++p) {
+      if (done[p]) continue;
+      if (it >= 2 && poll_end(2 * p + ((it - 1) & 1)) == 0) {
+        done[p] = true;
+        c->counters[6]--;
+        continue;
+      }
+      rounds_done[p] = it + 1;
+      if (it + 1 >= max_iters) poll_end(2 * p + (it & 1));
+    }
+  }
+  for (int p = 0; p < 2; ++p) {
+    int& expect = c->proj_rounds[dir[p]];
+    int& stable = c->proj_stable[dir[p]];
+    if (stopped[p] && rounds_done[p] < expect) rounds_done[p] = expect;
+    stable = rounds_done[p] == expect ? stable + 1 : 0;
+    expect = rounds_done[p];
+    enter(p);
+    if (sy.B > 0) launch(KNewtonEnd{c->w, iters_dst[p]}, sy.B);
+  }
+  enter(0);
   c->round = 0;
   return 0;
 }
@@ -1329,7 +1467,7 @@
       sp.order = ctx->d_order_ident;
       CHMC_FWD_PAR(ctx->plan.nld_waves, (long)sy.B, sp, ctx->sl, ctx->w, 0, 1, 0, 2, 1, 0);
     } else if (ctx->plan.nld == FwdWave)
-      launch_blocks(k_fwd_scan<M, RM, true>, ((long)sy.B + 63) / 64, 64 * (1 + CHMC_SCAN_HELPERS), 7, sf, ctx->sl, ctx->w, 0, 1, 0, 2);
+      launch_blocks(k_fwd_scan<M, RM, true>, ((long)sy.B + 63) / 64, 64 * (1 + CHMC_SCAN_HELPERS), 7, sf, ctx->sl, ctx->w, 0, 1, 0, 2, ctx->w, 0, 0);
     else
       launch(KFullScan<M>{sy, ctx->w.qb, ctx->w.trajw, QH}, sy.B, 7);
     launch_wave(k_nld_grad_wave<M>, (long)sy.B, 0, sy, ctx->w.qb, ctx->w.trajw, QH, use_gaussian_splitting, ctx->d_ham,
@@ -1482,8 +1620,11 @@
 static int step_enqueue(chmc_ctx* ctx, const double* dt, const int* active, const int* active_dev, int n_inner, int newton,
                         double ctol, double ptol, double dtol, int max_iters, double rev_tol,
                         const int* n_steps_host = nullptr, int n_steps_all = 1, bool want_n_done = false,
-                        bool skip_end_kick = false, bool pending_kick = false) {
-  const Sys& sy = ctx->sy;
+                        bool skip_end_kick = false, bool pending_kick = false, bool pair_next = false) {
+  const Sys& sy = ctx->sy;
+  const bool adopt = pending_kick && ctx->pair_ready;
+  ctx->pair_ready = false;
+  if (pair_next) pair_alloc(ctx);
   const double* d_dt = nullptr;
   if (ctx->last_dt.size() != (size_t)sy.B || ctx->last_n_inner != n_inner ||
       memcmp(ctx->last_dt.data(), dt, sizeof(double) * sy.B) != 0) {
@@ -1558,15 +1699,22 @@
       if (i > 0) {
         launch_rows(KFlow{sy, ctx->sl, ctx->w, 0, 0, 0, 1.0}, sy.Q, sy.B, 8);
       } else if (ctx->mom_tangent) {
-        if (pending_kick) launch_rows(KKick2FlowPg{sy, ctx->sl, ctx->w, kick}, sy.Q, sy.B, 8);
-        else launch_rows(KKickFlowPg{sy, ctx->sl, ctx->w, kick}, sy.Q, sy.B, 8);
+        if (adopt) {
+          launch_rows(KPairAdopt{sy, ctx->sl, ctx->w, kick, ctx->pw.qb}, sy.Q, sy.B, 8);
+          launch(KPairAdoptStatus{ctx->w, ctx->pw, ctx->d_itf, ctx->d_itf_next}, sy.B);
+        } else if (pending_kick) {
+          launch_rows(KKick2FlowPg{sy, ctx->sl, ctx->w, kick}, sy.Q, sy.B, 8);
+        } else {
+          launch_rows(KKickFlowPg{sy, ctx->sl, ctx->w, kick}, sy.Q, sy.B, 8);
+        }
       } else {
         launch(KKick{sy, ctx->sl, ctx->w, 0, 1, kick}, (long)sy.B * sy.Q, 8);
         project_momentum(ctx, 0, 3, 2);
         launch_rows(KFlow{sy, ctx->sl, ctx->w, 0, 0, 1, 1.0}, sy.Q, sy.B, 8);
       }
     }
-    run_projection(ctx, newton, 0, 0, ctol, ptol, dtol, max_iters, two ? &full : nullptr, 0);
+    if (!adopt)
+      run_projection(ctx, newton, 0, 0, ctol, ptol, dtol, max_iters, two ? &full : nullptr, 0);
     for (int h = 0; h < nh; ++h) {
       enter(h);
       state_eval_core(ctx, 1, last, 3);
@@ -1577,11 +1725,19 @@
         launch_rows(KMomFixInitPg{sy, ctx->sl, ctx->w, 1}, sy.Q, sy.B, 8);
       const bool flow_in_update = last && ctx->plan.rev_flow_in_update;
       if (last)
-        project_momentum_and_kick_direction(ctx, 1, false, fix_in_jw, flow_in_update);
+        project_momentum_and_kick_direction(ctx, 1, false, fix_in_jw, flow_in_update, pair_next ? ctx->pw.qb : nullptr, kick);
       else
         project_momentum(ctx, 1, 0, 0);
       launch_rows(KFlow{sy, ctx->sl, ctx->w, 1, 1, 0, -1.0}, flow_in_update ? sy.U : sy.Q, sy.B, 8);
-    }
+      if (pair_next) {
+        launch(KPairBegin{ctx->w, ctx->pw, ctx->d_itf_next}, sy.B);
+        launch_rows(KPairFlow{sy, ctx->sl, ctx->w, kick, ctx->pw.qb}, flow_in_update ? sy.U : sy.Q, sy.B, 8);
+      }
+    }
+    if (pair_next) {
+      run_projection_pair(ctx, newton, ctol, ptol, dtol, max_iters);
+      ctx->pair_ready = true;
+    } else
     run_projection(ctx, newton, 1, 1, ctol, ptol, dtol, max_iters, two ? &full : nullptr, 1);
     for (int h = 0; h < nh; ++h) {
       enter(h);
@@ -1701,8 +1857,9 @@
     for (int c = 0; c < B; ++c) any = (run[c] = act[c] && left[c] > 0) || any;
     if (!any) break;
     const bool skip = fuse_kicks && ctx->mom_tangent && k + 1 < longest;
+    const bool pair = skip && ctx->halves == 1 && pair_this_call(ctx->plan, ctx->plan_in.wave_kernels, B, sy.K, ctx->num_cus);
     if (step_enqueue(ctx, dt, run.data(), nullptr, n_inner, newton, ctol, ptol, dtol, max_iters, rev_tol, nullptr, 1, false, skip,
-                     pending))
+                     pending, pair))
       return -1;
     pending = skip;
     step_finish(ctx, true, n_inner, st.data(), f.data(), b.data(), r1.data());
diff --git a/manifold_mcmc_for_diffusions_amd/csrc/chmc_core.h b/manifold_mcmc_for_diffusions_amd/csrc/chmc_core.h
--- a/manifold_mcmc_for_diffusions_amd/csrc/chmc_core.h
+++ b/manifold_mcmc_for_diffusions_amd/csrc/chmc_core.h
@@ -1515,16 +1515,33 @@
   Work w;
   int which, qsel, psel;
   int flow_rev = 0;
-  CHMC_HD void rev_flow2(int c, int s, size_t i, double px, double py) const {
+  double* fwd_qb = nullptr;
+  double fwd_hfrac = 0.0;
+  CHMC_HD void rev_flow2(int c, int s, size_t i, double px, double py, double gx, double gy) const {
     const double2_ q0 = ld2_stream(pick(sl.q, s) + i);
     const double dt = -1.0 * w.dt[c];
     double2_ qn;
     qn.x = q0.x + dt * px, qn.y = q0.y + dt * py;
     stv2(w.qb + i, qn, true, true);
-  }
-  CHMC_HD void rev_flow1(int c, int s, size_t i, double px) const {
+    if (fwd_qb) {
+      const double h = fwd_hfrac * w.dt[c];
+      double2_ p1, p0, qf;
+      p1.x = px - h * gx, p1.y = py - h * gy;
+      p0.x = p1.x - h * gx, p0.y = p1.y - h * gy;
+      qf.x = q0.x + w.dt[c] * p0.x, qf.y = q0.y + w.dt[c] * p0.y;
+      stv2(fwd_qb + i, qf, true, true);
+    }
+  }
+  CHMC_HD void rev_flow1(int c, int s, size_t i, double px, double gx) const {
     const double dt = -1.0 * w.dt[c];
-    w.qb[i] = pick(sl.q, s)[i] + dt * px;
+    const double q0 = pick(sl.q, s)[i];
+    w.qb[i] = q0 + dt * px;
+    if (fwd_qb) {
+      const double h = fwd_hfrac * w.dt[c];
+      const double p1 = px - h * gx;
+      const double p0 = p1 - h * gx;
+      fwd_qb[i] = q0 + w.dt[c] * p0;
+    }
   }
   CHMC_HD bool active(int c) const {
     int p_ = 0, q_ = 0;
@@ -1610,7 +1627,7 @@
           if (TGT == 3) {
             o.x = old2[e * V], o.y = old2[e * V + V - 1];
             *reinterpret_cast<double2_*>(tgt2 + to + e * V) = o;
-            if (flow_rev) rev_flow2(c, s, off + to + e * V, o.x, o.y);
+            if (flow_rev) rev_flow2(c, s, off + to + e * V, o.x, o.y, old[e * V], old[e * V + V - 1]);
           }
         } else {
           CHMC_UNROLL
@@ -1618,7 +1635,7 @@
             tgt[to + e * V + k] = old[e * V + k];
             if (TGT == 3) {
               tgt2[to + e * V + k] = old2[e * V + k];
-              if (flow_rev) rev_flow1(c, s, off + to + e * V + k, old2[e * V + k]);
+              if (flow_rev) rev_flow1(c, s, off + to + e * V + k, old2[e * V + k], old[e * V + k]);
             }
           }
         }
@@ -1652,11 +1669,12 @@
         }
       }
       if (TGT == 0) r = absbits(d);
-      tgt[col] -= d;
+      const double gn = tgt[col] - d;
+      tgt[col] = gn;
       if (TGT == 3) {
         const double pn = tgt2[col] - d2;
         tgt2[col] = pn;
-        if (flow_rev) rev_flow1(c, s, off + col, pn);
+        if (flow_rev) rev_flow1(c, s, off + col, pn, gn);
       }
     }
     return r;
@@ -2003,6 +2021,20 @@
     stv2(pick(sl.p, s ^ 1) + i, pn, wide, two);
   }
 };
+CHMC_FI CHMC_HD inline void kick2_flow(const Sys& sy, const Work& w, int c, double h, const double2_& q0, const double2_& pp,
+                                const double2_& g, double2_& p1, double2_& qn, double2_& pn) {
+  double2_ p0;
+  p1.x = pp.x - h * g.x, p1.y = pp.y - h * g.y;
+  p0.x = p1.x - h * g.x, p0.y = p1.y - h * g.y;
+  if (sy.gaussian) {
+    const double sn = w.sdt[c], cs = w.cdt[c];
+    qn.x = q0.x * cs + sn * p0.x, qn.y = q0.y * cs + sn * p0.y;
+    pn.x = p0.x * cs - sn * q0.x, pn.y = p0.y * cs - sn * q0.y;
+  } else {
+    qn.x = q0.x + w.dt[c] * p0.x, qn.y = q0.y + w.dt[c] * p0.y;
+    pn = p0;
+  }
+}
 struct KKick2FlowPg {
   Sys sy;
   Slots sl;
@@ -2016,20 +2048,74 @@
     const bool two = col + 1 < sy.Q, wide = two && !(sy.Q & 1);
     const double2_ q0 = ldv2(pick(sl.q, s) + i, wide, two), pp = ldv2(pick(sl.p, s) + i, wide, two);
     const double2_ g = ldv2(pick(sl.pg, s) + i, wide, two);
-    double2_ p1, p0, qn, pn;
-    p1.x = pp.x - h * g.x, p1.y = pp.y - h * g.y;
-    p0.x = p1.x - h * g.x, p0.y = p1.y - h * g.y;
-    if (sy.gaussian) {
-      const double sn = w.sdt[c], cs = w.cdt[c];
-      qn.x = q0.x * cs + sn * p0.x, qn.y = q0.y * cs + sn * p0.y;
-      pn.x = p0.x * cs - sn * q0.x, pn.y = p0.y * cs - sn * q0.y;
-    } else {
-      qn.x = q0.x + w.dt[c] * p0.x, qn.y = q0.y + w.dt[c] * p0.y;
-      pn = p0;
-    }
+    double2_ p1, qn, pn;
+    kick2_flow(sy, w, c, h, q0, pp, g, p1, qn, pn);
     stv2(pick(sl.p, s) + i, p1, wide, two);
     stv2(pick(sl.q, s ^ 1) + i, qn, wide, two);
     stv2(pick(sl.p, s ^ 1) + i, pn, wide, two);
+  }
+};
+struct KPairBegin {
+  Work w, w2;
+  int* itf_next;
+  CHMC_HD void operator()(int c) const {
+    w2.ok[c] = w.ok[c];
+    w2.status[c] = w.ok[c] ? 0 : -1;
+    itf_next[c] = 0;
+  }
+};
+struct KPairFlow {
+  Sys sy;
+  Slots sl;
+  Work w;
+  double hfrac;
+  double* qf;
+  CHMC_HD bool active(int c) const { return w.ok[c] != 0; }
+  CHMC_FI CHMC_HD void operator()(int c, int col) const {
+    const int s = sl.cur[c] ^ 1;
+    const double h = hfrac * w.dt[c];
+    const size_t i = (size_t)c * sy.Q + col;
+    const bool two = col + 1 < sy.Q, wide = two && !(sy.Q & 1);
+    const double2_ q0 = ldv2(pick(sl.q, s) + i, wide, two), pp = ldv2(pick(sl.p, s) + i, wide, two);
+    const double2_ g = ldv2(pick(sl.pg, s) + i, wide, two);
+    double2_ p1, qn, pn;
+    kick2_flow(sy, w, c, h, q0, pp, g, p1, qn, pn);
+    stv2(qf + i, qn, wide, two);
+  }
+};
+struct KPairAdopt {
+  Sys sy;
+  Slots sl;
+  Work w;
+  double hfrac;
+  const double* qf;
+  CHMC_HD bool active(int c) const { return w.ok[c] != 0; }
+  CHMC_FI CHMC_HD void operator()(int c, int col) const {
+    const int s = sl.cur[c];
+    const double h = hfrac * w.dt[c];
+    const size_t i = (size_t)c * sy.Q + col;
+    const bool two = col + 1 < sy.Q, wide = two && !(sy.Q & 1);
+    double2_ q0;
+    q0.x = q0.y = 0.0;
+    if (sy.gaussian) q0 = ldv2(pick(sl.q, s) + i, wide, two);
+    const double2_ pp = ldv2(pick(sl.p, s) + i, wide, two), g = ldv2(pick(sl.pg, s) + i, wide, two);
+    const double2_ qc = ldv2(qf + i, wide, two);
+    double2_ p1, qn, pn;
+    kick2_flow(sy, w, c, h, q0, pp, g, p1, qn, pn);
+    stv2(pick(sl.p, s) + i, p1, wide, two);
+    stv2(pick(sl.q, s ^ 1) + i, qc, wide, two);
+    stv2(pick(sl.p, s ^ 1) + i, pn, wide, two);
+  }
+};
+struct KPairAdoptStatus {
+  Work w, w2;
+  int* itf;
+  const int* itf_next;
+  CHMC_HD void operator()(int c) const {
+    itf[c] = w.ok[c] ? itf_next[c] : 0;
+    if (!w.ok[c]) return;
+    w.iters[c] = w2.iters[c], w.nstat[c] = w2.nstat[c];
+    if (!w2.ok[c]) w.ok[c] = 0, w.status[c] = w2.status[c];
   }
 };
 struct KRevDiff {
diff --git a/manifold_mcmc_for_diffusions_amd/csrc/chmc_plan.h b/manifold_mcmc_for_diffusions_amd/csrc/chmc_plan.h
--- a/manifold_mcmc_for_diffusions_amd/csrc/chmc_plan.h
+++ b/manifold_mcmc_for_diffusions_amd/csrc/chmc_plan.h
@@ -19,7 +19,7 @@
   bool compact_rows = true, gram_mfma = false;
   int par_scan = kSwitchUnset, par_waves = kSwitchUnset, row_split = 0, halves = 1;
   bool no_fwd_scan = false, step_fusions = true;
-  int retract_kernel = kSwitchUnset;
+  int retract_kernel = kSwitchUnset, pair_retract = kSwitchUnset;
 };
 inline Switches read_switches() {
   auto env = [](const char* name, int unset) {
@@ -33,6 +33,7 @@
   s.row_split = env("CHMC_ROW_SPLIT", 0), s.halves = env("CHMC_HALVES", 1);
   s.no_fwd_scan = getenv("CHMC_NO_FWD_SCAN") != nullptr, s.step_fusions = env("CHMC_STEP_FUSIONS", 1) != 0;
   s.retract_kernel = env("CHMC_RETRACT_KERNEL", kSwitchUnset);
+  s.pair_retract = env("CHMC_PAIR_RETRACT", kSwitchUnset);
   return s;
 }
 
@@ -102,6 +103,8 @@
   bool mom_fix_in_jp;
   bool rev_flow_in_update;
   int retract_kernel;
+  bool pair_retractions;
+  int pair_retract;
   PartitionPlan part[2];
 };
 
@@ -135,6 +138,9 @@
   pl.mom_fix_in_jp = step_fusions && in.V == 2 && in.even_dims;
   pl.rev_flow_in_update = step_fusions && !in.gaussian;
   pl.retract_kernel = in.call.retract_kernel;
+  pl.pair_retract = in.call.pair_retract;
+  pl.pair_retractions = in.call.pair_retract != 0 && sw.halves != 2 && pl.fwd != FwdPar &&
+                        (!in.wave_kernels || pl.fwd_cold == FwdWave || in.call.pair_retract == 1);
 
   for (int p = 0; p < in.num_partition; ++p) {
     PartitionPlan& pp = pl.part[p];
@@ -157,6 +163,7 @@
     pp.rebuild_rows = compact && (!rows16 || ivl16);
     pp.retract_chain = compact && rows16 && K == 1;
     pp.traj_chain = pp.retract_chain && ivl16;
+    if (pp.retract_chain) pl.pair_retractions = false;
   }
   return pl;
 }
@@ -168,4 +175,10 @@
   return want == 1 ? CHMC_RETRACT_WAVES : want == 2 ? 4 : 0;
 }
 
+inline bool pair_this_call(const KernelPlan& pl, bool wave_kernels, int B, int K, int num_cus) {
+  if (!pl.pair_retractions) return false;
+  if (pl.pair_retract == 1 || !wave_kernels) return true;
+  return 2 * (((long)B * K + 63) / 64) <= num_cus;
 }
+
+}
diff --git a/manifold_mcmc_for_diffusions_amd/csrc/chmc_wave.h b/manifold_mcmc_for_diffusions_amd/csrc/chmc_wave.h
--- a/manifold_mcmc_for_diffusions_amd/csrc/chmc_wave.h
+++ b/manifold_mcmc_for_diffusions_amd/csrc/chmc_wave.h
@@ -4432,9 +4432,14 @@
 #ifndef CHMC_SCAN_HELPERS
 #define CHMC_SCAN_HELPERS 1
 #endif
-template <class M, int RM, bool STORE>
+template <class M, int RM, bool STORE, bool PAIR = false>
 __global__ void __launch_bounds__(STORE ? 64 * (1 + CHMC_SCAN_HELPERS) : 64)
-    k_fwd_scan(Sys sy, Slots sl, Work w, int which, int qsel, int use_nw, int store_traj) {
+    k_fwd_scan(Sys sy, Slots sl, Work w0, int which0, int qsel0, int use_nw, int store_traj, Work w1, int which1, int qsel1) {
+  const int wg0 = (sy.B * sy.K + 63) / 64;
+  const bool second = PAIR && (int)blockIdx.x >= wg0;
+  const Work w = second ? w1 : w0;
+  int which = second ? which1 : which0, qsel = second ? qsel1 : qsel0;
+  const int wg = second ? (int)blockIdx.x - wg0 : (int)blockIdx.x;
   constexpr int X = M::X, V = M::V, PF = 8;
   constexpr int NLD = PF * V / 2;
   constexpr int NST = PF * X / 2;
@@ -4457,7 +4462,7 @@
   const bool helper = STORE && wave_id != 0;
   const int hid = wave_id - 1;
   const int n = sy.B * sy.K, S = sy.S;
-  const int tid0 = blockIdx.x * 64;
+  const int tid0 = wg * 64;
 
   int maxL = 0;
   {
```

Result: faster. 54110 steps/s (median of 6 runs) (+4.1%).
